# nvpro-samples/vk_gltf_renderer

Measured on AMD Instinct MI355X. Metric: Msamples/s (and ms/frame @ fixed spp) 1080p & 4K, 1/2/4/8 MI355X, higher is better.
Workload: dtype f32

## Files before the change

### include/mi_pt.h

```cpp
#ifndef MI_PT_H
#define MI_PT_H

#include "mi_pt_shaderio.h"

#ifdef __cplusplus
extern "C" {
#endif

#if defined(__GNUC__)
#define MI_PT_API __attribute__((visibility("default")))
#else
#define MI_PT_API
#endif

typedef enum MiPtStatus
{
  MI_PT_OK            = 0,
  MI_PT_ERR_ARGUMENT  = -1,
  MI_PT_ERR_NO_DEVICE = -2,
  MI_PT_ERR_HIP       = -3,
  MI_PT_ERR_STATE     = -4,
  MI_PT_ERR_IO        = -5
} MiPtStatus;

// ... 92 lines not shown
  int   bounceIterations;
  float tracePrimaryMs;
  float shadeFirstMs;
  int   tracePrimaryLaunches;
  int   shadeFirstLaunches;
} MiPtFrameTiming;

typedef struct MiPt MiPt;

MI_PT_API int mi_pt_create(const MiPtSceneDesc* scene, const MiPtCreateOptions* options, MiPt** out);

MI_PT_API int mi_pt_update_render_nodes(MiPt* pt, const MiGltfRenderNode* renderNodes, int numRenderNodes, const uint8_t* renderNodeVisible);

MI_PT_API int mi_pt_update_lights(MiPt* pt, const MiGltfLight* lights, int numLights);

MI_PT_API int mi_pt_update_materials(MiPt* pt, const MiGltfShadeMaterial* materials, int numMaterials, const MiGltfTextureInfo* textureInfos,
                                     int numTextureInfos);

typedef struct MiPtDeformPrimitive
{
  int32_t         renderPrimID;
  uint32_t        vertexCount;
  const float*    basePositions;
  const float*    baseNormals;
  const float*    baseTangents;
  const uint16_t* joints;
  const float*    weights;
  uint32_t        numJoints;
  uint32_t        jointMatrixOffset;
  uint32_t        numTargets;
  uint32_t        morphWeightOffset;
  const float*    positionDeltas;
  const float*    normalDeltas;
  const float*    tangentDeltas;
} MiPtDeformPrimitive;

typedef struct MiPtDeformDesc
{
  const MiPtDeformPrimitive* prims;
  int                        numPrims;
  int                        numJointMatrices;
  int                        numMorphWeights;
  const float*               jointMatrices;
  const float*               morphWeights;
} MiPtDeformDesc;

enum { MI_PT_DEFORM_DEFER_BUILD = 1 };

MI_PT_API int mi_pt_set_deformation(MiPt* pt, const MiPtDeformDesc* desc);
MI_PT_API int mi_pt_update_deformation(MiPt* pt, const float* jointMatrices, const float* morphWeights, int flags);
enum
{
  MI_PT_ACCEL_REBUILD = 0,
  MI_PT_ACCEL_REFIT   = 1,
  MI_PT_ACCEL_AUTO    = 2
};
enum { MI_PT_ACCEL_LAST_BUILD = 0, MI_PT_ACCEL_LAST_REFIT = 1 };
MI_PT_API int mi_pt_set_accel_update(MiPt* pt, int mode, float rebuildCostRatio);
typedef struct MiPtAccelInfo
{
  int32_t  mode;
  int32_t  lastUpdate;
  float    rebuildCostRatio;
  int32_t  reserved;
  uint64_t builds;
  uint64_t refits;
  double   sahCostAtBuild;
  double   sahCost;
  uint64_t trianglesMoved;
  uint64_t refitBytes;
} MiPtAccelInfo;
MI_PT_API int mi_pt_get_accel_info(MiPt* pt, MiPtAccelInfo* info);
MI_PT_API int mi_pt_set_accel_resident(MiPt* pt, int enable);
typedef struct MiPtAccelResidentInfo
{
  int32_t  enabled;
  int32_t  inForce;
  uint64_t residentTriangles;
  uint64_t hiddenTriangles;
  uint64_t visibilityRefits;
  uint64_t materialPatches;
} MiPtAccelResidentInfo;
MI_PT_API int mi_pt_get_accel_resident_info(MiPt* pt, MiPtAccelResidentInfo* info);
MI_PT_API int mi_pt_read_vertices(MiPt* pt, int renderPrimID, float* positions, float* normals, float* tangents);

MI_PT_API int mi_pt_destroy(MiPt* pt);

MI_PT_API int mi_pt_set_environment(MiPt* pt, const MiPtEnvironment* env);

MI_PT_API int mi_pt_resize(MiPt* pt, int width, int height);

MI_PT_API int mi_pt_set_frame_info(MiPt* pt, const MiSceneFrameInfo* info);
MI_PT_API int mi_pt_set_sky(MiPt* pt, const MiSkyPhysicalParameters* sky);

MI_PT_API int mi_pt_set_tile_partition(MiPt* pt, int rank, int world, int tileSize);

MI_PT_API int mi_pt_bind_accum(MiPt* pt, void* deviceRGBA32F);
MI_PT_API int mi_pt_bind_guides(MiPt* pt, void* deviceAlbedoRGBA32F, void* deviceNormalRGBA32F, void* deviceDepthR32F);

MI_PT_API int mi_pt_render_frame(MiPt* pt, const MiPathtraceParams* params, void* hipStream);

MI_PT_API int mi_pt_render_frames(MiPt* pt, const MiPathtraceParams* params, int numFrames, void* hipStream);

MI_PT_API int mi_pt_set_frame_queue(MiPt* pt, int depth);

MI_PT_API int mi_pt_synchronize(MiPt* pt);

MI_PT_API int mi_pt_read_accum(MiPt* pt, float* hostRGBA32F);
MI_PT_API int mi_pt_write_accum(MiPt* pt, const float* hostRGBA32F);
MI_PT_API int mi_pt_read_guides(MiPt* pt, float* hostAlbedoRGBA32F, float* hostNormalRGBA32F);
MI_PT_API int mi_pt_read_selection(MiPt* pt, uint32_t* hostObjectIds);
MI_PT_API int mi_pt_read_depth(MiPt* pt, float* hostDepth);
MI_PT_API void* mi_pt_accum_device_ptr(MiPt* pt);

MI_PT_API int mi_pt_denoise(MiPt* pt, int iterations, float sigmaColor, float sigmaNormal, float sigmaAlbedo,
                            float* hostRGBA32F, void* hipStream);

MI_PT_API int mi_pt_denoise_svgf(MiPt* pt, int iterations, float sigmaLuminance, float sigmaNormal, float sigmaDepth, float* hostRGBA32F, void* hipStream);


MI_PT_API int mi_pt_read_first_hit(MiPt* pt, float* hostXYZW);
MI_PT_API int mi_pt_set_temporal(MiPt* pt, int enable);
MI_PT_API int mi_pt_read_motion(MiPt* pt, float* hostRGBA32F);
typedef struct MiPtTemporalParams
{
  int   iterations;
  float sigmaLuminance;
  float sigmaNormal;
  float sigmaDepth;
  float alpha;
  float momentsAlpha;
  float maxHistory;
  float normalCos;
  float depthTolerance;
} MiPtTemporalParams;
MI_PT_API void mi_pt_default_temporal(MiPtTemporalParams* params);
MI_PT_API int mi_pt_denoise_temporal(MiPt* pt, const MiPtTemporalParams* params, float* hostRGBA32F, void* hipStream);
MI_PT_API int mi_pt_reset_history(MiPt* pt);

MI_PT_API int mi_pt_set_vertex_motion(MiPt* pt, int enable);
MI_PT_API int mi_pt_read_first_hit_triangle(MiPt* pt, uint32_t* hostPrimTriB1B2);
MI_PT_API int mi_pt_read_previous_positions(MiPt* pt, int renderPrimID, float* positions);

enum { MI_PT_VERTICES_RECOMPUTE_NORMALS = 1 };
typedef struct MiPtVertexUpdate
{
  int32_t      renderPrimID;
  uint32_t     vertexCount;
  const float* positions;
  const float* normals;
  const float* tangents;
  uint32_t     reserved[2];
} MiPtVertexUpdate;
MI_PT_API int mi_pt_set_vertex_updates(MiPt* pt, const int32_t* renderPrimIDs, int count, int flags);
MI_PT_API int mi_pt_update_vertices(MiPt* pt, const MiPtVertexUpdate* updates, int numUpdates, int flags);
MI_PT_API int mi_pt_update_vertices_device(MiPt* pt, const MiPtVertexUpdate* updates, int numUpdates, int flags);
typedef struct MiPtVertexUpdateInfo
{
  uint64_t calls;
  uint64_t verticesWritten;
  uint64_t verticesRejected;
  uint64_t tableBytes;
} MiPtVertexUpdateInfo;
MI_PT_API int mi_pt_get_vertex_update_info(MiPt* pt, MiPtVertexUpdateInfo* info);

typedef struct MiPtRay
// ... 83 lines not shown
```

### vk_gltf_renderer_amd/_capi.py

```python
import ctypes as C
import os
from enum import IntEnum

_HERE = os.path.dirname(os.path.abspath(__file__))
LIB_DIR = os.path.join(_HERE, "lib")

f32 = C.c_float
i32 = C.c_int
u32 = C.c_uint32


class MiGltfRenderNode(C.Structure):
    _fields_ = [("objectToWorld", f32 * 16), ("worldToObject", f32 * 16), ("materialID", i32), ("renderPrimID", i32)]


class MiGltfLight(C.Structure):
    _fields_ = [("direction", f32 * 3), ("type", i32), ("position", f32 * 3), ("radius", f32), ("color", f32 * 3),
                ("intensity", f32), ("angularSizeOrInvRange", f32), ("innerAngle", f32), ("outerAngle", f32), ("_pad", i32)]


class MiGltfTextureInfo(C.Structure):
    _fields_ = [("uvTransform", f32 * 6), ("index", i32), ("texCoord", i32)]


# ... 43 lines not shown
                ("sunGlowIntensity", f32), ("yIsUp", i32)]


class MiEnvAccel(C.Structure):
    _fields_ = [("alias", u32), ("q", f32)]


class MiTonemapperData(C.Structure):
    _fields_ = [("method", i32), ("isActive", i32), ("exposure", f32), ("brightness", f32), ("contrast", f32), ("saturation", f32), ("vignette", f32),
                ("autoExposure", i32), ("autoExposureSpeed", f32), ("evMinValue", f32), ("evMaxValue", f32), ("enableCenterMetering", i32)]


TONEMAP_METHODS = ("filmic", "uncharted", "clip", "aces", "agx", "khronos_pbr")


class MiPtRenderPrimitive(C.Structure):
    _fields_ = [("indices", C.POINTER(u32)), ("triangleCount", u32), ("vertexCount", u32), ("positions", C.POINTER(f32)),
                ("normals", C.POINTER(f32)), ("colors", C.POINTER(u32)), ("tangents", C.POINTER(f32)),
                ("texCoords0", C.POINTER(f32)), ("texCoords1", C.POINTER(f32)), ("opaqueTriangleCount", u32), ("reserved", u32)]


class MiPtTexture(C.Structure):
    _fields_ = [("levels", C.POINTER(C.POINTER(C.c_uint8))), ("width", i32), ("height", i32), ("numLevels", i32),
                ("srgb", i32), ("magFilter", i32), ("minFilter", i32), ("mipmapMode", i32), ("wrapS", i32), ("wrapT", i32)]


class MiPtSceneDesc(C.Structure):
    _fields_ = [("materials", C.POINTER(MiGltfShadeMaterial)), ("numMaterials", i32),
                ("textureInfos", C.POINTER(MiGltfTextureInfo)), ("numTextureInfos", i32),
                ("renderNodes", C.POINTER(MiGltfRenderNode)), ("numRenderNodes", i32),
                ("renderNodeVisible", C.POINTER(C.c_uint8)),
                ("renderPrimitives", C.POINTER(MiPtRenderPrimitive)), ("numRenderPrimitives", i32),
                ("lights", C.POINTER(MiGltfLight)), ("numLights", i32),
                ("textures", C.POINTER(MiPtTexture)), ("numTextures", i32)]


class MiPtEnvironment(C.Structure):
    _fields_ = [("rgba", C.POINTER(f32)), ("accel", C.POINTER(MiEnvAccel)), ("width", i32), ("height", i32), ("integral", f32)]


class MiPtCreateOptions(C.Structure):
    _fields_ = [("device", i32), ("collectCounters", i32), ("bvhBuilder", i32), ("reserved", i32 * 5)]


class MiPtStats(C.Structure):
    _fields_ = [(n, C.c_uint64) for n in (
        "cameraPaths", "segments", "shadowRays", "nodesClosest", "trisClosest", "nodesShadow", "trisShadow",
        "textureTaps", "bvhNodeCount", "bvhTriangleCount", "bvhNodeBytes", "bvhTriangleBytes", "surfaceHits", "nodesPrimary", "trisPrimary")]


class MiPtMemory(C.Structure):
    _fields_ = [(n, C.c_uint64) for n in ("sceneBytes", "rendererBytes", "deviceUsedBytes", "deviceTotalBytes", "pathStateBytes", "pathSlots")]


class MiPtFrameTiming(C.Structure):
    _fields_ = [("totalMs", f32), ("generateMs", f32), ("traceClosestMs", f32), ("sortMs", f32), ("shadeMs", f32),
                ("traceShadowMs", f32), ("accumulateMs", f32), ("traceClosestLaunches", i32), ("shadeLaunches", i32),
                ("traceShadowLaunches", i32), ("bounceIterations", i32), ("tracePrimaryMs", f32), ("shadeFirstMs", f32),
                ("tracePrimaryLaunches", i32), ("shadeFirstLaunches", i32)]


class MiPtDeformPrimitive(C.Structure):
    _fields_ = [("renderPrimID", i32), ("vertexCount", u32), ("basePositions", C.POINTER(f32)), ("baseNormals", C.POINTER(f32)),
                ("baseTangents", C.POINTER(f32)), ("joints", C.POINTER(C.c_uint16)), ("weights", C.POINTER(f32)), ("numJoints", u32),
                ("jointMatrixOffset", u32), ("numTargets", u32), ("morphWeightOffset", u32), ("positionDeltas", C.POINTER(f32)),
                ("normalDeltas", C.POINTER(f32)), ("tangentDeltas", C.POINTER(f32))]


class MiPtDeformDesc(C.Structure):
    _fields_ = [("prims", C.POINTER(MiPtDeformPrimitive)), ("numPrims", i32), ("numJointMatrices", i32), ("numMorphWeights", i32),
                ("jointMatrices", C.POINTER(f32)), ("morphWeights", C.POINTER(f32))]


class MiPtAccelInfo(C.Structure):
    _fields_ = [("mode", i32), ("lastUpdate", i32), ("rebuildCostRatio", f32), ("reserved", i32), ("builds", C.c_uint64), ("refits", C.c_uint64),
                ("sahCostAtBuild", C.c_double), ("sahCost", C.c_double), ("trianglesMoved", C.c_uint64), ("refitBytes", C.c_uint64)]


class MiPtAccelResidentInfo(C.Structure):
    _fields_ = [("enabled", i32), ("inForce", i32), ("residentTriangles", C.c_uint64), ("hiddenTriangles", C.c_uint64),
                ("visibilityRefits", C.c_uint64), ("materialPatches", C.c_uint64)]


class MiPtTemporalParams(C.Structure):
    _fields_ = [("iterations", i32), ("sigmaLuminance", f32), ("sigmaNormal", f32), ("sigmaDepth", f32), ("alpha", f32), ("momentsAlpha", f32),
                ("maxHistory", f32), ("normalCos", f32), ("depthTolerance", f32)]


class MiPtRay(C.Structure):
    _fields_ = [("origin", f32 * 3), ("tMin", f32), ("direction", f32 * 3), ("tMax", f32)]


class MiPtRayHit(C.Structure):
    _fields_ = [("t", f32), ("b1", f32), ("b2", f32), ("flags", u32), ("renderNode", i32), ("renderPrimID", i32), ("triangle", u32),
                ("materialID", i32), ("position", f32 * 3), ("reserved0", f32), ("normal", f32 * 3), ("reserved1", f32)]


class MiPtQueryOptions(C.Structure):
    _fields_ = [("mode", i32), ("alpha", i32), ("cull", i32), ("maxHits", i32), ("blendThreshold", f32), ("seed", u32), ("reserved", i32 * 2)]


class MiPtVertexUpdate(C.Structure):
    _fields_ = [("renderPrimID", i32), ("vertexCount", u32), ("positions", C.c_void_p), ("normals", C.c_void_p), ("tangents", C.c_void_p),
                ("reserved", u32 * 2)]


class MiPtVertexUpdateInfo(C.Structure):
    _fields_ = [(n, C.c_uint64) for n in ("calls", "verticesWritten", "verticesRejected", "tableBytes")]


class MiCamera(C.Structure):
    _fields_ = [("eye", f32 * 3), ("center", f32 * 3), ("up", f32 * 3), ("fovDegrees", f32), ("znear", f32),
                ("zfar", f32), ("orthographic", i32), ("xmag", f32), ("ymag", f32)]


assert C.sizeof(MiGltfRenderNode) == 136
assert C.sizeof(MiGltfLight) == 64
assert C.sizeof(MiGltfTextureInfo) == 32
assert C.sizeof(MiGltfShadeMaterial) == 288
assert C.sizeof(MiSceneFrameInfo) == 396
assert C.sizeof(MiPtAccelInfo) == 64
assert C.sizeof(MiPtAccelResidentInfo) == 40
assert C.sizeof(MiPtRay) == 32
assert C.sizeof(MiPtRayHit) == 64
assert C.sizeof(MiPtQueryOptions) == 32
assert C.sizeof(MiPtVertexUpdate) == 40
assert C.sizeof(MiPtVertexUpdateInfo) == 32

MI_PT_ABI_VERSION = 9
MI_PT_DEFORM_DEFER_BUILD = 1
MI_PT_VERTICES_RECOMPUTE_NORMALS = 1
(MI_SCENE_CHANGED_NODES, MI_SCENE_CHANGED_LIGHTS, MI_SCENE_CHANGED_DEFORMATION, MI_SCENE_CHANGED_MATERIALS, MI_SCENE_CHANGED_CAMERAS,
 MI_SCENE_CHANGED_VISIBILITY) = 1, 2, 4, 8, 16, 32
MI_PT_ACCEL_REBUILD, MI_PT_ACCEL_REFIT, MI_PT_ACCEL_AUTO = 0, 1, 2
MI_PT_ACCEL_LAST_BUILD, MI_PT_ACCEL_LAST_REFIT = 0, 1
MI_PT_HIT, MI_PT_HIT_FRONT_FACE, MI_PT_HIT_INVALID_RAY = 1, 2, 4
MI_PT_QUERY_CLOSEST, MI_PT_QUERY_ANY, MI_PT_QUERY_NEAREST_K = 0, 1, 2
MI_PT_QUERY_ALPHA_OPAQUE, MI_PT_QUERY_ALPHA_CUTOFF, MI_PT_QUERY_ALPHA_STOCHASTIC = 0, 1, 2
MI_PT_QUERY_CULL_NONE, MI_PT_QUERY_CULL_MATERIAL = 0, 1
MI_PT_QUERY_MAX_HITS = 8
MI_PT_CAMERA_RAYS_UNIT = 1
MI_PROJECTION_PERSPECTIVE, MI_PROJECTION_EQUIRECT, MI_PROJECTION_FISHEYE = 0, 1, 2
MI_PT_USE_DLSS, MI_PT_USE_OPTIX_DENOISER, MI_PT_FIRST_FRAME = 1, 2, 4
MI_SCENE_IS_ORTHOGRAPHIC, MI_SCENE_USE_SOLID_BACKGROUND, MI_SCENE_USE_HDR_ENVIRONMENT = 1, 2, 4
MI_SCENE_USE_INFINITE_PLANE, MI_SCENE_INFINITE_PLANE_SHADOW_CATCHER = 8, 16
MI_LIGHT_NONE, MI_LIGHT_DIRECTIONAL, MI_LIGHT_SPOT, MI_LIGHT_POINT = 0, 1, 2, 3


class Visualization(IntEnum):
    RENDERED = 0
    BASE_COLOR = 1
    METALLIC = 2
    ROUGHNESS = 3
    NORMAL_SHADING = 4
    NORMAL_GEOMETRIC = 5
    TANGENT = 6
    BITANGENT = 7
    EMISSIVE = 8
    OPACITY = 9
    TEXCOORD0 = 10
    TEXCOORD1 = 11
    CLAY = 12
    TRIANGLE_ID = 13
    FACE_ORIENTATION = 14
    OCCLUSION = 15
    CLEARCOAT_FACTOR = 16
    CLEARCOAT_ROUGHNESS = 17
    CLEARCOAT_NORMAL = 18
    SHEEN_COLOR = 19
    SHEEN_ROUGHNESS = 20
    SPECULAR_FACTOR = 21
    SPECULAR_COLOR = 22
    TRANSMISSION_FACTOR = 23
    IRIDESCENCE_FACTOR = 24
    IRIDESCENCE_THICKNESS = 25
    ANISOTROPY_STRENGTH = 26
    DIFFUSE_TRANSMISSION_FACTOR = 27
    DIFFUSE_TRANSMISSION_COLOR = 28
    OPACITY_MICROMAP = 29


MI_VIZ_COUNT = 30

P = C.POINTER
VP = C.c_void_p

HOST_SYMBOLS = {
    "mi_scene_load": (i32, [C.c_char_p, P(VP)]),
    "mi_scene_destroy": (None, [VP]),
    "mi_scene_desc": (P(MiPtSceneDesc), [VP]),
    "mi_scene_num_cameras": (i32, [VP]),
    "mi_scene_camera": (i32, [VP, i32, P(MiCamera)]),
    "mi_scene_bounds": (None, [VP, P(f32), P(f32)]),
    "mi_scene_num_triangles": (C.c_uint64, [VP]),
    "mi_hdr_load": (i32, [C.c_char_p, P(VP)]),
    "mi_scene_recompute_tangents": (i32, [VP, i32, i32]),
    "mi_mikktspace": (i32, [P(f32), P(f32), P(f32), u32, P(u32), u32, P(f32)]),
    "mi_scene_cut_alpha": (C.c_int64, [VP, i32]),
    "mi_scene_num_variants": (i32, [VP]),
    "mi_scene_variant_name": (i32, [VP, i32, C.c_char_p, i32]),
    "mi_scene_current_variant": (i32, [VP]),
    "mi_scene_set_variant": (i32, [VP, i32]),
    "mi_scene_num_animations": (i32, [VP]),
    "mi_scene_animation_info": (i32, [VP, i32, P(f32), P(f32), C.c_char_p, i32]),
    "mi_scene_update_animation": (i32, [VP, i32, f32]),
    "mi_scene_animation_changes": (i32, [VP]),
    "mi_scene_deformation": (P(MiPtDeformDesc), [VP]),
    "mi_scene_deform_on_host": (i32, [VP]),
    "mi_hdr_from_pixels": (i32, [i32, i32, P(f32), P(VP)]),
    "mi_hdr_destroy": (None, [VP]),
    "mi_hdr_env": (P(MiPtEnvironment), [VP]),
    "mi_default_sky": (None, [P(MiSkyPhysicalParameters)]),
    "mi_default_params": (None, [P(MiPathtraceParams)]),
    "mi_camera_frame_info": (None, [P(MiCamera), i32, i32, P(MiSceneFrameInfo), P(f32), P(f32)]),
    "mi_camera_rays": (i32, [P(MiCamera), i32, f32, i32, i32, P(f32), i32, P(MiPtRay), P(f32)]),
    "mi_host_last_error": (C.c_char_p, []),
}

PT_SYMBOLS = {
    "mi_pt_create": (i32, [P(MiPtSceneDesc), P(MiPtCreateOptions), P(VP)]),
    "mi_pt_destroy": (i32, [VP]),
    "mi_pt_set_environment": (i32, [VP, P(MiPtEnvironment)]),
    "mi_pt_resize": (i32, [VP, i32, i32]),
    "mi_pt_set_frame_info": (i32, [VP, P(MiSceneFrameInfo)]),
    "mi_pt_set_sky": (i32, [VP, P(MiSkyPhysicalParameters)]),
    "mi_pt_set_tile_partition": (i32, [VP, i32, i32, i32]),
    "mi_pt_bind_accum": (i32, [VP, VP]),
    "mi_pt_bind_guides": (i32, [VP, VP, VP, VP]),
    "mi_pt_render_frame": (i32, [VP, P(MiPathtraceParams), VP]),
    "mi_pt_render_frames": (i32, [VP, P(MiPathtraceParams), i32, VP]),
    "mi_pt_synchronize": (i32, [VP]),
    "mi_pt_read_accum": (i32, [VP, P(f32)]),
    "mi_pt_write_accum": (i32, [VP, P(f32)]),
    "mi_pt_read_guides": (i32, [VP, P(f32), P(f32)]),
    "mi_pt_read_selection": (i32, [VP, P(u32)]),
    "mi_pt_read_depth": (i32, [VP, P(f32)]),
    "mi_pt_set_frame_queue": (i32, [VP, i32]),
    "mi_pt_accum_device_ptr": (VP, [VP]),
    "mi_pt_denoise": (i32, [VP, i32, f32, f32, f32, P(f32), VP]),
    "mi_pt_denoise_svgf": (i32, [VP, i32, f32, f32, f32, P(f32), VP]),
    "mi_pt_denoised_device_ptr": (VP, [VP]),
    "mi_pt_tonemap": (i32, [VP, P(MiTonemapperData), i32, f32, P(C.c_uint8), VP]),
    "mi_pt_tonemapped_device_ptr": (VP, [VP]),
    "mi_pt_default_tonemapper": (None, [P(MiTonemapperData), i32]),
    "mi_pt_get_memory": (i32, [VP, P(MiPtMemory)]),
    "mi_pt_get_stats": (i32, [VP, P(MiPtStats)]),
    "mi_pt_reset_stats": (i32, [VP]),
    "mi_pt_enable_timing": (i32, [VP, i32]),
    "mi_pt_get_frame_timing": (i32, [VP, P(MiPtFrameTiming)]),
    "mi_pt_last_error": (C.c_char_p, []),
    "mi_pt_version": (C.c_char_p, []),
    "mi_pt_abi_version": (i32, []),
    "mi_pt_update_render_nodes": (i32, [VP, P(MiGltfRenderNode), i32, P(C.c_uint8)]),
    "mi_pt_update_lights": (i32, [VP, P(MiGltfLight), i32]),
    "mi_pt_update_materials": (i32, [VP, P(MiGltfShadeMaterial), i32, P(MiGltfTextureInfo), i32]),
    "mi_pt_set_deformation": (i32, [VP, P(MiPtDeformDesc)]),
    "mi_pt_update_deformation": (i32, [VP, P(f32), P(f32), i32]),
    "mi_pt_read_vertices": (i32, [VP, i32, P(f32), P(f32), P(f32)]),
    "mi_pt_set_accel_update": (i32, [VP, i32, f32]),
    "mi_pt_get_accel_info": (i32, [VP, P(MiPtAccelInfo)]),
    "mi_pt_set_accel_resident": (i32, [VP, i32]),
    "mi_pt_get_accel_resident_info": (i32, [VP, P(MiPtAccelResidentInfo)]),
    "mi_pt_read_first_hit": (i32, [VP, P(f32)]),
    "mi_pt_set_temporal": (i32, [VP, i32]),
    "mi_pt_read_motion": (i32, [VP, P(f32)]),
    "mi_pt_default_temporal": (None, [P(MiPtTemporalParams)]),
    "mi_pt_denoise_temporal": (i32, [VP, P(MiPtTemporalParams), P(f32), VP]),
    "mi_pt_reset_history": (i32, [VP]),
    "mi_pt_set_vertex_motion": (i32, [VP, i32]),
    "mi_pt_read_first_hit_triangle": (i32, [VP, P(u32)]),
    "mi_pt_read_previous_positions": (i32, [VP, i32, P(f32)]),
    "mi_pt_query_rays": (i32, [VP, P(MiPtRay), i32, i32, P(MiPtRayHit)]),
    "mi_pt_query_rays_device": (i32, [VP, VP, i32, i32, VP, VP]),
    "mi_pt_pick": (i32, [VP, P(f32), i32, P(MiPtRayHit)]),
    "mi_pt_default_query_options": (None, [P(MiPtQueryOptions)]),
    "mi_pt_query_rays_ex": (i32, [VP, P(MiPtRay), i32, P(MiPtQueryOptions), P(MiPtRayHit)]),
    "mi_pt_query_rays_device_ex": (i32, [VP, VP, i32, P(MiPtQueryOptions), VP, VP]),
    "mi_pt_pick_ex": (i32, [VP, P(f32), i32, P(MiPtQueryOptions), P(MiPtRayHit)]),
    "mi_pt_set_vertex_updates": (i32, [VP, P(i32), i32, i32]),
    "mi_pt_update_vertices": (i32, [VP, P(MiPtVertexUpdate), i32, i32]),
    "mi_pt_update_vertices_device": (i32, [VP, P(MiPtVertexUpdate), i32, i32]),
    "mi_pt_get_vertex_update_info": (i32, [VP, P(MiPtVertexUpdateInfo)]),
    "mi_pt_set_camera_rays": (i32, [VP, P(MiPtRay), i32, u32]),
    "mi_pt_set_camera_rays_device": (i32, [VP, VP, i32, u32]),
    "mi_pt_make_camera_rays": (i32, [VP, P(MiPathtraceParams), i32, P(MiPtRay)]),
    "mi_pt_make_camera_rays_device": (i32, [VP, P(MiPathtraceParams), i32, VP, VP]),
}


def _bind(lib, table):
    for name, (res, args) in table.items():
        fn = getattr(lib, name)
        fn.restype = res
        fn.argtypes = args
    return lib


_host = None
_pt = None


def host_lib():
    global _host
    if _host is None:
        path = os.path.join(LIB_DIR, "libmi_host.so")
        if not os.path.exists(path):
            raise RuntimeError(f"{path} is missing: run __graft_entry__.build() (make -C vk_gltf_renderer_amd/csrc)")
        _host = _bind(C.CDLL(path), HOST_SYMBOLS)
    return _host


def pt_lib():
    global _pt
    if _pt is None:
        path = os.environ.get("MI_PT_LIB") or os.path.join(LIB_DIR, "libmi_pt.so")
        if not os.path.exists(path):
            raise RuntimeError(f"{path} is missing: the HIP extension was not built; the product path has no fallback")
        _pt = _bind(C.CDLL(path), PT_SYMBOLS)
        if _pt.mi_pt_abi_version() != MI_PT_ABI_VERSION:
            raise RuntimeError(f"{path}: ABI version {_pt.mi_pt_abi_version()}, this binding was written for {MI_PT_ABI_VERSION}")
    return _pt


def device_source_id():
    import glob
    import hashlib
    root = os.path.dirname(_HERE)
    dev = os.path.join(_HERE, "csrc", "device")
    files = sorted(glob.glob(os.path.join(dev, "*.hip")) + glob.glob(os.path.join(dev, "*.h")), key=os.path.basename)
    files += [os.path.join(root, "include", "mi_pt.h"), os.path.join(root, "include", "mi_pt_shaderio.h")]
    h = hashlib.sha1()
    for f in files:
        h.update(open(f, "rb").read())
    return h.hexdigest()[:16]
```

### vk_gltf_renderer_amd/csrc/device/mi_pt_api.hip

```cpp
#include <hip/hip_runtime.h>

#include <algorithm>
#include <chrono>
#include <cstdlib>
#include <cmath>
#include <cstdio>
#include <cstring>
#include <memory>
#include <string>
#include <vector>

#include "mi_pt.h"
#include "bvh_refit.h"
#include "dev_buf.h"
#include "material_patch.h"
#include "pt_build.h"
#include "pt_bvh.h"
#include "pt_deform.h"
#include "pt_vertex_update.h"
#include "pt_kernels.h"
#include "pt_query.h"

namespace {

thread_local std::string g_lastError;

int fail(int code, const std::string& msg)
{
  g_lastError = msg;
  return code;
}

#define HIP_TRY(x)                                                                                                       \
  do                                                                                                                    \
  {                                                                                                                     \
    hipError_t e_ = (x);                                                                                                \
    if(e_ != hipSuccess)                                                                                                \
      return fail(MI_PT_ERR_HIP, std::string(#x) + ": " + hipGetErrorString(e_));                                       \
  } while(0)

using pt::DevBuf;

enum TimedKernel { TK_GENERATE, TK_TRACE, TK_SORT, TK_SHADE, TK_SHADOW, TK_ACCUM, TK_PRIMARY, TK_SHADE_FIRST, TK_COUNT };

}

struct RunSwitches
{
  int    packetInterval = 1;
  int    sortMode       = 2;
  bool   noPacket       = false;
  bool   stateBySlot    = false;
  bool   traceSpans     = false;
  int    overlapUpTo    = 32;
  int    overlapMinTris = 200000;
  bool   noPlanes       = false;
  bool   noOpaqueTris   = false;
  bool   noQuads        = false;
  bool   shadowFarFirst = true;
  int    reinsert       = 16;
  int    reinsertUpdate = 0;
  int    reinsertRounds = 4;
  float  splitFactor    = 4.0f;
  int    splitMaxDepth  = 8;
  float  splitMinShare  = 0.1f;
  bool   collapseGreedy = false;
  bool   collapseBad    = false;
  bool   hostCollapse   = false;
  bool   coreTex        = true;
  bool   shadowDeposit  = true;
  int    maxItersDiag   = 0;
  int    failBuildAt    = 0;
  bool   candPoolSet    = false;
  size_t candPool       = 0;
  void   read()
  {
    auto flag = [](const char* n) { const char* e = getenv(n); return e != nullptr; };
    auto num  = [](const char* n, int d) { const char* e = getenv(n); return e ? atoi(e) : d; };
    packetInterval = num("MI_PT_PACKET_INTERVAL", 1);
    sortMode       = num("MI_PT_SORT", 2);
    noPacket       = flag("MI_PT_NO_PACKET");
    stateBySlot    = flag("MI_PT_STATE_BY_SLOT");
    traceSpans     = flag("MI_PT_TRACE_SPANS");
    overlapUpTo    = num("MI_PT_OVERLAP", 32);
    overlapMinTris = num("MI_PT_OVERLAP_MIN_TRIS", 200000);
    noPlanes       = flag("MI_PT_DIAG_NO_PLANES");
    noOpaqueTris   = flag("MI_PT_DIAG_NO_OPAQUE_TRIS");
    noQuads        = flag("MI_PT_DIAG_NO_QUADS");
    shadowFarFirst = num("MI_PT_SHADOW_FAR_FIRST", 1) != 0;
    reinsert       = std::max(0, num("MI_PT_REINSERT", 16));
    reinsertUpdate = std::max(0, num("MI_PT_REINSERT_UPDATE", 0));
    reinsertRounds = std::max(1, num("MI_PT_REINSERT_ROUNDS", 4));
    if(const char* e = getenv("MI_PT_SPLIT"))
      splitFactor = std::max(0.0f, float(atof(e)));
    if(const char* e = getenv("MI_PT_SPLIT_MIN_SHARE"))
      splitMinShare = std::max(0.0f, float(atof(e)));
    splitMaxDepth  = std::min(std::max(0, num("MI_PT_SPLIT_DEPTH", 8)), 10);
    if(const char* e = getenv("MI_PT_COLLAPSE"))
    {
      collapseGreedy = strcmp(e, "greedy") == 0;
      collapseBad    = !collapseGreedy && strcmp(e, "sah") != 0;
    }
    hostCollapse   = flag("MI_PT_HOST_COLLAPSE");
    maxItersDiag   = num("MI_PT_DIAG_MAX_ITERS", 0);
    coreTex        = num("MI_PT_CORE_TEX", 1) != 0;
    shadowDeposit  = num("MI_PT_SHADOW_DEPOSIT", 1) != 0;
    failBuildAt    = num("MI_PT_DIAG_FAIL_BUILD", 0);
    if(const char* e = getenv("MI_PT_DIAG_CAND_POOL"))
    {
      candPoolSet = true;
      candPool    = size_t(strtoull(e, nullptr, 10));
    }
  }
};

struct MiPt
{
  int device = 0;
  int numCUs = 256;
  RunSwitches sw;
  int accelBuilds = 0;
  int               frameQueueDepth = 1;
  int               pendingFrames   = 0;
  MiPathtraceParams pendingFirst{};
  void*             pendingStream   = nullptr;
  DevBuf<MiGltfShadeMaterial> materials;
  DevBuf<MiGltfTextureInfo>   texInfos;
  DevBuf<pt::DevTexRef>       texRefs;
  DevBuf<pt::DevCoreTex>      coreTex;
  DevBuf<MiGltfRenderNode>    nodes;
  DevBuf<pt::DevPrim>         prims;
  DevBuf<MiGltfLight>         lights;
  DevBuf<pt::DevTexture>      textures;
  DevBuf<uchar4>              texels;
  DevBuf<uint4>               texQuads;
  DevBuf<uint8_t>             geometry;
  DevBuf<uint8_t>             instFlags;
  DevBuf<float>               srgbLut;
  DevBuf<float4>              envPixels;
  DevBuf<MiEnvAccel>          envAccel;
  DevBuf<pt::DevAlphaTri>     alphaTris;
  DevBuf<pt::DevShadeTri>     shadeTris;
  DevBuf<float4>              bvhNodes;
  DevBuf<uint4>               bvh8Nodes;
  DevBuf<float>               bvh8Planes;
  DevBuf<pt::DevTri>          bvhTris;
  bool                        wide      = true;
  pt::DevScene                scene{};
  bool                        hasAlpha = false, hasAlphaTest = false, hasVolumeScatter = false, simpleMaterials = true, hasTransmissive = false;
  static constexpr int        FC_RING = 32;
  DevBuf<pt::DevScene>        sceneDev;
  bool                        sceneDevDirty = true;
  DevBuf<pt::FrameConsts>     fcRing;
  DevBuf<pt::SkyPrecomp>      skyPre;
  MiSkyPhysicalParameters     skyPreFor{};
  bool                        skyPreValid = false;
  pt::FrameConsts*            fcHost = nullptr;
  hipEvent_t                  fcDone[FC_RING] = {};
  unsigned                    fcCursor = 0;
  MiPtStats                   staticStats{};
  std::vector<MiGltfRenderNode> hostNodes;
  std::vector<uint8_t>          hostVisible;
  std::vector<uint8_t>          matInstFlags;
  std::vector<uint8_t>          matFeatures;
  std::vector<MiGltfShadeMaterial> hostMaterials;
  std::vector<MiGltfTextureInfo>   hostTexInfos;
  std::vector<pt::DevTexture>      hostTextures;
  DevBuf<uint8_t>               matDirty;
  bool                          splitRefs = false;
  std::vector<uint32_t>         primTriangles;
  std::vector<pt::DevPrim>      hostPrims;
  std::vector<uint32_t>         primVertices;
  DevBuf<uint8_t>               deformPool;
  DevBuf<pt::DeformTask>        deformTasks;
  DevBuf<uint32_t>              deformBlockTask;
  DevBuf<float4>                deformJoints;
  DevBuf<float>                 deformWeights;
  int                           deformJointCount = 0, deformWeightCount = 0;
  uint32_t                      deformBlocks = 0;
  bool                          deformSet = false;
  std::vector<int>              deformPrimIDs;
  bool                          vuSet = false;
  std::vector<int>              vuPrimIDs;
  std::vector<uint8_t>          vuDeclared;
  std::vector<size_t>           vuCornerEnd, vuCorners;
  DevBuf<uint32_t>              vuTable;
  DevBuf<pt::VertexUpdateTask>  vuTasks;
  DevBuf<pt::NormalRebuildTask> vuNormalTasks;
  DevBuf<uint32_t>              vuBlockTask;
  size_t                        vuBlockCap = 0;
  DevBuf<uint8_t>               vuStaging;
  uint64_t                      vuCalls = 0, vuWritten = 0, vuRejected = 0;
  int                           bvhBuilder = 0;
  int                           accelMode = MI_PT_ACCEL_REBUILD;
  float                         accelRatio = 1.5f;
  int                           lastUpdate = MI_PT_ACCEL_LAST_BUILD;
  bool                          switchBuild = false;
  bool                          refitCapable = false;
  uint64_t                      accelRefits = 0, trianglesMoved = 0;
  double                        sahAtBuild = 0.0, sahNow = 0.0;
  DevBuf<pt::RefitBox>          refitSlotBox, refitBuiltBox, refitNodeBox;
  DevBuf<float>                 refitSah;
  DevBuf<double>                refitSahPartial;
  DevBuf<uint8_t>               refitDirty;
  std::vector<uint32_t>         refitLevels;
  std::vector<MiGltfRenderNode> builtNodes;
  std::vector<uint8_t>          primDirty;
  std::vector<uint8_t>          primDeformed;
  bool                          accelResident = false;
  bool                          residentTree  = false;
  uint64_t                      hiddenTris = 0;
  uint64_t                      visibilityRefits = 0, materialPatches = 0;
  int                     width = 0, height = 0;
  int                     tileRank = 0, tileWorld = 1, tileSize = 64;
  MiSceneFrameInfo        frameInfo{};
  MiSkyPhysicalParameters sky{};
  bool                    haveFrameInfo = false;
  DevBuf<uint32_t>        ownedTiles;
  int                     numSlots = 0, tilesX = 0, tilesY = 0;
  int                     framesCap = 1;
  size_t                  queueCap  = 0;
  DevBuf<float4>          pathArrays;
  DevBuf<float4>          optThroughput, optMisc, optMedium, optPixelSum, optGuides, optShadowAux2;
  DevBuf<float4>          firstHit;
  pt::PathSoA             paths{};
  DevBuf<uint32_t>        queueMem;
  DevBuf<float4>          queuePayload;
  DevBuf<float4>          candPool;
  DevBuf<uint32_t>        candLists;
  pt::Queues              queues{};
  DevBuf<float4>          accumOwn, albedo, normal, denoiseA, denoiseB;
  float4*                 albedoBound = nullptr;
// ... 1049 lines not shown
          if(p.normals) { o[3] = p.normals[3 * size_t(v)]; o[4] = p.normals[3 * size_t(v) + 1]; o[5] = p.normals[3 * size_t(v) + 2]; }
          if(p.texCoords0) { o[6] = p.texCoords0[2 * size_t(v)]; o[7] = p.texCoords0[2 * size_t(v) + 1]; }
          if(p.tangents) memcpy(o + 8, p.tangents + 4 * size_t(v), 16);
        }
        d.verts = reinterpret_cast<const float4*>(put(iv.data(), iv.size() * sizeof(float)));
      }
    }
    HIP_TRY(hipMemcpy(pt->geometry.ptr, staging.data(), staging.size(), hipMemcpyHostToDevice));
  }
  HIP_TRY(pt->prims.upload(devPrims.data(), devPrims.size()));
  pt->hostPrims = devPrims;
  for(int i = 0; i < sd->numRenderPrimitives; ++i)
    pt->primVertices.push_back(sd->renderPrimitives[i].vertexCount);
  phase("tables + geometry upload");

  pt->hostNodes.assign(sd->renderNodes, sd->renderNodes + sd->numRenderNodes);
  if(sd->renderNodeVisible)
    pt->hostVisible.assign(sd->renderNodeVisible, sd->renderNodeVisible + sd->numRenderNodes);
  pt->matInstFlags.resize(size_t(sd->numMaterials));
  pt->matFeatures.resize(size_t(sd->numMaterials));
  pt->hostMaterials.assign(sd->materials, sd->materials + sd->numMaterials);
  pt->hostTexInfos.assign(sd->textureInfos, sd->textureInfos + sd->numTextureInfos);
  for(int m = 0; m < sd->numMaterials; ++m)
  {
    pt->matInstFlags[size_t(m)] = materialInstFlags(sd->materials[m]);
    pt->matFeatures[size_t(m)]  = materialFeatures(sd->materials[m]);
  }
  pt->primTriangles.resize(size_t(sd->numRenderPrimitives));
  for(int i = 0; i < sd->numRenderPrimitives; ++i)
  {
    const MiPtRenderPrimitive& rp = sd->renderPrimitives[i];
    pt->primTriangles[size_t(i)]  = (rp.positions && rp.indices) ? rp.triangleCount : 0u;
  }
  pt->bvhBuilder = options ? options->bvhBuilder : 0;

  {
    std::vector<pt::DevTexture> dt(size_t(sd->numTextures));
    size_t                      totalTexels = 0;
    for(int i = 0; i < sd->numTextures; ++i)
    {
      const MiPtTexture& t = sd->textures[i];
      if(t.numLevels < 1 || t.numLevels > 16 || t.width < 1 || t.height < 1 || t.width > 65535 || t.height > 65535)
        return fail(MI_PT_ERR_ARGUMENT, "mi_pt_create: texture dimensions / level count out of range");
      for(int l = 0; l < t.numLevels; ++l)
        totalTexels += size_t(std::max(1, t.width >> l)) * size_t(std::max(1, t.height >> l));
    }
    if(totalTexels > 0xffffffffull)
      return fail(MI_PT_ERR_ARGUMENT, "mi_pt_create: texture pool exceeds 2^32 texels");
    std::vector<uchar4> pool(std::max<size_t>(totalTexels, 1));
    size_t              off = 0;
    for(int i = 0; i < sd->numTextures; ++i)
    {
      const MiPtTexture& t = sd->textures[i];
      pt::DevTexture&    d = dt[size_t(i)];
      memset(&d, 0, sizeof(d));
      d.width = uint16_t(t.width); d.height = uint16_t(t.height); d.numLevels = uint8_t(t.numLevels); d.srgb = uint8_t(t.srgb ? 1 : 0);
      d.magFilter = uint8_t(t.magFilter); d.minFilter = uint8_t(t.minFilter); d.mipmapMode = uint8_t(t.mipmapMode);
      d.wrapS = uint8_t(t.wrapS); d.wrapT = uint8_t(t.wrapT);
      for(int l = 0; l < t.numLevels; ++l)
      {
        size_t n         = size_t(std::max(1, t.width >> l)) * size_t(std::max(1, t.height >> l));
        d.levelOffset[l] = uint32_t(off);
        memcpy(&pool[off], t.levels[l], n * 4);
        off += n;
      }
    }
    HIP_TRY(pt->textures.upload(dt.data(), dt.size()));
    HIP_TRY(pt->texels.upload(pool.data(), pool.size()));
    if(totalTexels > 0 && !pt->sw.noQuads)
    {
      HIP_TRY(pt->texQuads.alloc(pool.size()));
      for(const pt::DevTexture& d : dt)
        for(int l = 0; l < d.numLevels; ++l)
          pt::launchTextureQuads(pt->texels.ptr, pt->texQuads.ptr, d.levelOffset[l], std::max(1, int(d.width) >> l), std::max(1, int(d.height) >> l), d.wrapS,
                                 d.wrapT, nullptr);
      HIP_TRY(hipGetLastError());
    }
    pt->hostTextures = dt;
    std::vector<pt::DevTexRef>  refs;
    std::vector<pt::DevCoreTex> core;
    deriveTextureRecords(pt.get(), sd->materials, sd->numMaterials, sd->textureInfos, sd->numTextureInfos, refs, core);
    HIP_TRY(pt->texRefs.upload(refs.data(), refs.size()));
    HIP_TRY(pt->coreTex.upload(core.data(), core.size()));
  }
  {
    float lut[256];
    for(int i = 0; i < 256; ++i)
    {
      float c = float(i) / 255.0f;
      lut[i]  = c <= 0.04045f ? c / 12.92f : std::pow((c + 0.055f) / 1.055f, 2.4f);
    }
    HIP_TRY(pt->srgbLut.upload(lut, 256));
  }
  phase("textures upload");

  pt::DevScene& S = pt->scene;
  S.materials = pt->materials.ptr; S.texInfos = pt->texInfos.ptr; S.nodes = pt->nodes.ptr; S.prims = pt->prims.ptr; S.lights = pt->lights.ptr;
  S.textures = pt->textures.ptr; S.texels = pt->texels.ptr; S.texQuads = pt->texQuads.ptr; S.envPixels = nullptr; S.envAccel = nullptr; S.bvhNodes = nullptr; S.bvh8Nodes = nullptr; S.bvh8Planes = nullptr; S.tris = nullptr;
  S.geomPool = reinterpret_cast<const float4*>(pt->geometry.ptr);
  S.texRefs = pt->texRefs.ptr; S.coreTex = reinterpret_cast<const uint4*>(pt->coreTex.ptr); S.alphaTris = nullptr; S.shadeTris = nullptr; S.srgbLut = pt->srgbLut.ptr; S.numMaterials = sd->numMaterials; S.numTextures = sd->numTextures;
  S.numLights = sd->numLights; S.numNodes = sd->numRenderNodes;
  S.envWidth = 0; S.envHeight = 0;
  S.packetInterval = pt->sw.packetInterval;
  S.shadowOctFlip  = pt->sw.shadowFarFirst ? 7u : 0u;
  if(int rc = buildAcceleration(pt.get()))
    return rc;
  phase("shade / alpha records");
  HIP_TRY(pt->stats.alloc(1));
  HIP_TRY(hipMemset(pt->stats.ptr, 0, sizeof(pt::StatCounters)));
  MiSkyPhysicalParameters s{};
  s.rgbUnitConversion[0] = s.rgbUnitConversion[1] = s.rgbUnitConversion[2] = 1.0f / 80000.0f;
  s.multiplier = 0.1f; s.haze = 0.1f; s.redblueshift = 0.1f; s.saturation = 1.0f; s.groundColor[0] = s.groundColor[1] = s.groundColor[2] = 0.4f;
  s.horizonBlur = 0.3f; s.sunDiskIntensity = 1.0f; s.sunDirection[0] = s.sunDirection[1] = s.sunDirection[2] = 0.5773502691896258f;
  s.sunDiskScale = 1.0f; s.sunGlowIntensity = 1.0f; s.yIsUp = 1;
  pt->sky = s;
  *out    = pt.release();
  return MI_PT_OK;
}

int mi_pt_update_render_nodes(MiPt* pt, const MiGltfRenderNode* renderNodes, int numRenderNodes, const uint8_t* renderNodeVisible)
{
  FLUSH_PENDING(pt);
  if(!pt || !renderNodes || numRenderNodes != int(pt->hostNodes.size()))
    return fail(MI_PT_ERR_ARGUMENT, "mi_pt_update_render_nodes: the render-node count must be the one the instance was created with");
  for(int n = 0; n < numRenderNodes; ++n)
    if(renderNodes[n].materialID >= int(pt->matInstFlags.size()))
      return fail(MI_PT_ERR_ARGUMENT, "mi_pt_update_render_nodes: render node references a material beyond the table");
  if(residentInForce(pt))
    return updateRenderNodesResident(pt, renderNodes, numRenderNodes, renderNodeVisible);
  HIP_TRY(hipSetDevice(pt->device));
  HIP_TRY(hipDeviceSynchronize());
  bool                 sameTopology = true;
  std::vector<uint8_t> moved(size_t(numRenderNodes), 0);
  for(int n = 0; n < numRenderNodes; ++n)
  {
    const MiGltfRenderNode &was = pt->hostNodes[size_t(n)], &now = renderNodes[n];
    const bool              visWas = pt->hostVisible.empty() || pt->hostVisible[size_t(n)], visNow = !renderNodeVisible || renderNodeVisible[n];
    if(was.materialID != now.materialID || was.renderPrimID != now.renderPrimID || visWas != visNow)
      sameTopology = false;
    moved[size_t(n)] = memcmp(was.objectToWorld, now.objectToWorld, sizeof(float) * 32) != 0;
  }
  pt->hostNodes.assign(renderNodes, renderNodes + numRenderNodes);
  if(renderNodeVisible)
    pt->hostVisible.assign(renderNodeVisible, renderNodeVisible + numRenderNodes);
  else
    pt->hostVisible.clear();
  return updateAcceleration(pt, sameTopology, moved);
}

int mi_pt_update_lights(MiPt* pt, const MiGltfLight* lights, int numLights)
{
  FLUSH_PENDING(pt);
  if(!pt || numLights != pt->scene.numLights || (numLights > 0 && !lights))
    return fail(MI_PT_ERR_ARGUMENT, "mi_pt_update_lights: the light count must be the one the instance was created with");
  if(numLights == 0)
    return MI_PT_OK;
  HIP_TRY(hipSetDevice(pt->device));
  HIP_TRY(hipDeviceSynchronize());
  HIP_TRY(hipMemcpy(pt->lights.ptr, lights, sizeof(MiGltfLight) * size_t(numLights), hipMemcpyHostToDevice));
  return MI_PT_OK;
}

int mi_pt_update_materials(MiPt* pt, const MiGltfShadeMaterial* materials, int numMaterials, const MiGltfTextureInfo* textureInfos, int numTextureInfos)
{
  FLUSH_PENDING(pt);
  if(!pt || !materials || !textureInfos || numMaterials != int(pt->hostMaterials.size()))
    return fail(MI_PT_ERR_ARGUMENT, "mi_pt_update_materials: the material count must be the one the instance was created with");
  if(numTextureInfos <= 0)
    return fail(MI_PT_ERR_ARGUMENT, "mi_pt_update_materials: the texture-info table needs the reserved slot 0");
  {
    std::string why;
    if(!materialSlotsInRange(materials, numMaterials, numTextureInfos, why))
      return fail(MI_PT_ERR_ARGUMENT, "mi_pt_update_materials: " + why);
  }
  const size_t         nm = size_t(numMaterials);
  std::vector<uint8_t> newFlags(nm), newFeatures(nm), alphaChanged(nm, 0), flagsChanged(nm, 0);
  bool                 anyAlpha = false, anyFlags = false, transmissiveChanged = false;
  for(size_t m = 0; m < nm; ++m)
  {
    newFlags[m]    = materialInstFlags(materials[m]);
    newFeatures[m] = materialFeatures(materials[m]);
    const AlphaKey was = alphaKey(pt->hostMaterials[m], pt->hostTexInfos.data()), now = alphaKey(materials[m], textureInfos);
    alphaChanged[m] = memcmp(&was, &now, sizeof(AlphaKey)) != 0;
    flagsChanged[m] = newFlags[m] != pt->matInstFlags[m];
    anyAlpha |= alphaChanged[m] != 0;
    anyFlags |= flagsChanged[m] != 0;
  }
  const int numNodes = int(pt->hostNodes.size()), numPrims = int(pt->hostPrims.size());
  auto      materialOf = [&](int n) { return size_t(std::max(0, std::min(pt->hostNodes[size_t(n)].materialID, numMaterials - 1))); };
  for(int n = 0; n < numNodes; ++n)
  {
    const size_t m    = materialOf(n);
    const int    prim = pt->hostNodes[size_t(n)].renderPrimID;
    if(alphaChanged[m] && prim >= 0 && prim < numPrims && pt->hostPrims[size_t(prim)].opaqueTriangles > 0)
      return fail(MI_PT_ERR_ARGUMENT, "mi_pt_update_materials: alpha state of a material whose geometry was cut at load: re-cut and re-create (material "
                                          + std::to_string(m) + ", render node " + std::to_string(n) + ")");
    if(((newFlags[m] ^ pt->matInstFlags[m]) & pt::INST_TRANSMISSIVE) != 0)
      transmissiveChanged = true;
  }
  HIP_TRY(hipSetDevice(pt->device));
  HIP_TRY(hipDeviceSynchronize());
  {
    std::vector<pt::DevTexRef>  refs;
    std::vector<pt::DevCoreTex> core;
    deriveTextureRecords(pt, materials, numMaterials, textureInfos, numTextureInfos, refs, core);
    if(size_t(numTextureInfos) != pt->texInfos.count)
    {
      DevBuf<MiGltfTextureInfo> infos;
      DevBuf<pt::DevTexRef>     drefs;
      HIP_TRY(infos.upload(textureInfos, size_t(numTextureInfos)));
      HIP_TRY(drefs.upload(refs.data(), refs.size()));
      std::swap(pt->texInfos.ptr, infos.ptr); std::swap(pt->texInfos.count, infos.count);
      std::swap(pt->texRefs.ptr, drefs.ptr); std::swap(pt->texRefs.count, drefs.count);
      pt->scene.texInfos = pt->texInfos.ptr;
      pt->scene.texRefs  = pt->texRefs.ptr;
    }
    else
    {
      HIP_TRY(hipMemcpy(pt->texInfos.ptr, textureInfos, sizeof(MiGltfTextureInfo) * size_t(numTextureInfos), hipMemcpyHostToDevice));
      HIP_TRY(hipMemcpy(pt->texRefs.ptr, refs.data(), sizeof(pt::DevTexRef) * refs.size(), hipMemcpyHostToDevice));
    }
    HIP_TRY(hipMemcpy(pt->materials.ptr, materials, sizeof(MiGltfShadeMaterial) * nm, hipMemcpyHostToDevice));
    HIP_TRY(hipMemcpy(pt->coreTex.ptr, core.data(), sizeof(pt::DevCoreTex) * core.size(), hipMemcpyHostToDevice));
  }
  pt->hostMaterials.assign(materials, materials + numMaterials);
  pt->hostTexInfos.assign(textureInfos, textureInfos + numTextureInfos);
  pt->matInstFlags = newFlags;
  pt->matFeatures  = newFeatures;
  pt->sceneDevDirty = true;
  const bool hadTransmissive = pt->hasTransmissive, wasSimple = pt->simpleMaterials;
  const std::vector<uint8_t> flags = instanceFlags(pt);
  if((anyAlpha || anyFlags) && pt->scene.numTris > 0 && (!pt->wide || (transmissiveChanged && pt->splitRefs)))
  {
    if(int rc = buildAcceleration(pt))
      return rc;
    return followSummaries(pt, hadTransmissive, wasSimple);
  }
  if(pt->scene.numTris > 0)
  {
    std::vector<uint8_t> dirty(size_t(std::max(numNodes, 1)), 0);
    for(int n = 0; n < numNodes; ++n)
    {
      const size_t m = materialOf(n);
      dirty[size_t(n)] = uint8_t((flagsChanged[m] ? pt::MATERIAL_PATCH_FLAGS : 0) | (alphaChanged[m] ? pt::MATERIAL_PATCH_ALPHA : 0));
    }
    if(int rc = patchTriangleData(pt, flags, dirty))
      return rc;
  }
  return followSummaries(pt, hadTransmissive, wasSimple);
}

static void releaseDeformation(MiPt* pt)
{
  pt->deformPool.release();
  pt->deformTasks.release();
  pt->deformBlockTask.release();
  pt->deformJoints.release();
  pt->deformWeights.release();
  pt->deformJointCount = pt->deformWeightCount = 0;
  pt->deformBlocks = 0;
  pt->deformSet    = false;
  pt->deformPrimIDs.clear();
}

int mi_pt_set_deformation(MiPt* pt, const MiPtDeformDesc* desc)
{
  FLUSH_PENDING(pt);
  if(!pt)
    return fail(MI_PT_ERR_ARGUMENT, "mi_pt_set_deformation: null instance");
  HIP_TRY(hipSetDevice(pt->device));
  HIP_TRY(hipDeviceSynchronize());
  if(!desc)
  {
    releaseDeformation(pt);
    return allocVertexMotion(pt);
  }
  const int numPrims = int(pt->primVertices.size());
  if(desc->numPrims < 0 || desc->numJointMatrices < 0 || desc->numMorphWeights < 0 || (desc->numPrims > 0 && !desc->prims))
    return fail(MI_PT_ERR_ARGUMENT, "mi_pt_set_deformation: negative count or null primitive table");
  std::vector<uint8_t> seen(size_t(numPrims), 0);
  size_t               poolBytes = 0;
  uint64_t             blocks    = 0;
  for(int k = 0; k < desc->numPrims; ++k)
  {
    const MiPtDeformPrimitive& d   = desc->prims[k];
    const std::string          who = "mi_pt_set_deformation: primitive " + std::to_string(k) + ": ";
    if(d.renderPrimID < 0 || d.renderPrimID >= numPrims)
      return fail(MI_PT_ERR_ARGUMENT, who + "render primitive " + std::to_string(d.renderPrimID) + " out of range");
    if(seen[size_t(d.renderPrimID)]++)
      return fail(MI_PT_ERR_ARGUMENT, who + "render primitive " + std::to_string(d.renderPrimID) + " listed twice");
    if(pt->vuSet && pt->vuDeclared[size_t(d.renderPrimID)])
      return fail(MI_PT_ERR_ARGUMENT, who + "render primitive " + std::to_string(d.renderPrimID) + " is driven by the caller (mi_pt_set_vertex_updates)");
    const pt::DevPrim& rp = pt->hostPrims[size_t(d.renderPrimID)];
    if(d.vertexCount != pt->primVertices[size_t(d.renderPrimID)])
      return fail(MI_PT_ERR_ARGUMENT, who + "vertexCount differs from the resident primitive's");
    if(!d.basePositions || !rp.positions)
      return fail(MI_PT_ERR_ARGUMENT, who + "no base positions");
    if((d.baseNormals && !rp.normals) || (d.baseTangents && !rp.tangents))
// ... 405 lines not shown
  if(!pt || !out)
    return fail(MI_PT_ERR_ARGUMENT, "mi_pt_get_vertex_update_info: null argument");
  out->calls            = pt->vuCalls;
  out->verticesWritten  = pt->vuWritten;
  out->verticesRejected = pt->vuRejected;
  out->tableBytes       = pt->vuTable.bytes();
  return MI_PT_OK;
}

int mi_pt_set_accel_update(MiPt* pt, int mode, float rebuildCostRatio)
{
  FLUSH_PENDING(pt);
  if(!pt)
    return fail(MI_PT_ERR_ARGUMENT, "mi_pt_set_accel_update: null instance");
  if(mode != MI_PT_ACCEL_REBUILD && mode != MI_PT_ACCEL_REFIT && mode != MI_PT_ACCEL_AUTO)
    return fail(MI_PT_ERR_ARGUMENT, "mi_pt_set_accel_update: unknown mode " + std::to_string(mode));
  if(!std::isfinite(rebuildCostRatio) || rebuildCostRatio < 1.0f)
    return fail(MI_PT_ERR_ARGUMENT, "mi_pt_set_accel_update: the rebuild cost ratio must be finite and at least 1");
  HIP_TRY(hipSetDevice(pt->device));
  HIP_TRY(hipDeviceSynchronize());
  pt->accelMode  = mode;
  pt->accelRatio = rebuildCostRatio;
  if(mode == MI_PT_ACCEL_REBUILD)
  {
    releaseRefitData(pt);
    return MI_PT_OK;
  }
  if(!pt->refitLevels.empty() || !pt->refitCapable)
    return MI_PT_OK;
  pt->switchBuild = true;
  const int rc    = buildAcceleration(pt);
  pt->switchBuild = false;
  return rc;
}

int mi_pt_get_accel_info(MiPt* pt, MiPtAccelInfo* out)
{
  if(!pt || !out)
    return fail(MI_PT_ERR_ARGUMENT, "mi_pt_get_accel_info: null argument");
  memset(out, 0, sizeof(*out));
  out->mode             = pt->accelMode;
  out->lastUpdate       = pt->lastUpdate;
  out->rebuildCostRatio = pt->accelRatio;
  out->builds           = uint64_t(std::max(pt->accelBuilds, 0));
  out->refits           = pt->accelRefits;
  out->sahCostAtBuild   = pt->sahAtBuild;
  out->sahCost          = pt->sahNow;
  out->trianglesMoved   = pt->trianglesMoved;
  out->refitBytes       = refitBytes(pt);
  return MI_PT_OK;
}

int mi_pt_set_accel_resident(MiPt* pt, int enable)
{
  FLUSH_PENDING(pt);
  if(!pt)
    return fail(MI_PT_ERR_ARGUMENT, "mi_pt_set_accel_resident: null instance");
  HIP_TRY(hipSetDevice(pt->device));
  HIP_TRY(hipDeviceSynchronize());
  pt->accelResident = enable != 0;
  if(residentWanted(pt) == pt->residentTree || pt->accelMode == MI_PT_ACCEL_REBUILD || (pt->bvhBuilder & 1) != 0 || pt->sw.hostCollapse)
    return MI_PT_OK;
  pt->switchBuild = true;
  const int rc    = buildAcceleration(pt);
  pt->switchBuild = false;
  return rc;
}

int mi_pt_get_accel_resident_info(MiPt* pt, MiPtAccelResidentInfo* out)
{
  if(!pt || !out)
    return fail(MI_PT_ERR_ARGUMENT, "mi_pt_get_accel_resident_info: null argument");
  memset(out, 0, sizeof(*out));
  const bool inForce     = residentInForce(pt);
  out->enabled           = pt->accelResident ? 1 : 0;
  out->inForce           = inForce ? 1 : 0;
  out->residentTriangles = inForce ? uint64_t(std::max(pt->scene.numTris, 0)) : 0;
  out->hiddenTriangles   = inForce ? pt->hiddenTris : 0;
  out->visibilityRefits  = pt->visibilityRefits;
  out->materialPatches   = pt->materialPatches;
  return MI_PT_OK;
}

int mi_pt_read_vertices(MiPt* pt, int renderPrimID, float* positions, float* normals, float* tangents)
{
  FLUSH_PENDING(pt);
  if(!pt || renderPrimID < 0 || renderPrimID >= int(pt->hostPrims.size()))
    return fail(MI_PT_ERR_ARGUMENT, "mi_pt_read_vertices: no such render primitive");
  HIP_TRY(hipSetDevice(pt->device));
  HIP_TRY(hipDeviceSynchronize());
  const pt::DevPrim& p  = pt->hostPrims[size_t(renderPrimID)];
  const size_t       nv = pt->primVertices[size_t(renderPrimID)];
  if(positions && p.positions && nv)
    HIP_TRY(hipMemcpy(positions, p.positions, nv * 12, hipMemcpyDeviceToHost));
  if(normals && p.normals && nv)
    HIP_TRY(hipMemcpy(normals, p.normals, nv * 12, hipMemcpyDeviceToHost));
  if(tangents && p.tangents && nv)
    HIP_TRY(hipMemcpy(tangents, p.tangents, nv * 16, hipMemcpyDeviceToHost));
  return MI_PT_OK;
}

int mi_pt_destroy(MiPt* pt)
{
  if(pt)
    pt->pendingFrames = 0;
  if(!pt)
    return MI_PT_OK;
  (void)hipSetDevice(pt->device);
  (void)hipDeviceSynchronize();
  pt::dumpTraceProfile();
  delete pt;
  return MI_PT_OK;
}

int mi_pt_set_environment(MiPt* pt, const MiPtEnvironment* env)
{
  FLUSH_PENDING(pt);
  if(!pt)
    return fail(MI_PT_ERR_ARGUMENT, "mi_pt_set_environment: null instance");
  HIP_TRY(hipSetDevice(pt->device));
  HIP_TRY(hipDeviceSynchronize());
  if(!env || !env->rgba || !env->accel || env->width <= 0 || env->height <= 0)
  {
    pt->envPixels.release();
    pt->envAccel.release();
    pt->scene.envPixels = nullptr;
    pt->scene.envAccel  = nullptr;
    pt->scene.envWidth = pt->scene.envHeight = 0;
    pt->sceneDevDirty  = true;
    return MI_PT_OK;
  }
  const size_t n = size_t(env->width) * size_t(env->height);
  HIP_TRY(pt->envPixels.upload(reinterpret_cast<const float4*>(env->rgba), n));
  HIP_TRY(pt->envAccel.upload(env->accel, n));
  pt->scene.envPixels = pt->envPixels.ptr;
  pt->scene.envAccel  = pt->envAccel.ptr;
  pt->scene.envWidth  = env->width;
  pt->scene.envHeight = env->height;
  pt->sceneDevDirty   = true;
  return MI_PT_OK;
}

int mi_pt_resize(MiPt* pt, int width, int height)
{
  FLUSH_PENDING(pt);
  if(!pt || width <= 0 || height <= 0 || width > 32768 || height > 32768)
    return fail(MI_PT_ERR_ARGUMENT, "mi_pt_resize: need 0 < width, height <= 32768");
  HIP_TRY(hipSetDevice(pt->device));
  HIP_TRY(hipDeviceSynchronize());
  pt->width       = width;
  pt->height      = height;
  pt->denoised    = nullptr;
  pt->accumFrames = 0.0f;
  pt->momentFrames = 0.0f;
  return allocFrameResources(pt);
}

int mi_pt_set_frame_info(MiPt* pt, const MiSceneFrameInfo* info)
{
  if(!pt || !info)
    return fail(MI_PT_ERR_ARGUMENT, "mi_pt_set_frame_info: null argument");
  if(pt->haveFrameInfo && memcmp(&pt->frameInfo, info, sizeof(*info)) == 0)
    return MI_PT_OK;
  FLUSH_PENDING(pt);
  pt->frameInfo     = *info;
  pt->haveFrameInfo = true;
// ... 108 lines not shown
    return fail(MI_PT_ERR_ARGUMENT, "mi_pt_render_frame: numSamples >= 1 and 1 <= maxDepth <= 255 required");
  if((pt->frameInfo.flags & MI_SCENE_USE_HDR_ENVIRONMENT) && !pt->scene.envPixels)
    return fail(MI_PT_ERR_STATE, "mi_pt_render_frame: HDR environment requested but none was set");
  if(cameraRaysStale(pt))
    return fail(MI_PT_ERR_STATE, CAMERA_RAYS_STALE);
  HIP_TRY(hipSetDevice(pt->device));
  hipStream_t stream = reinterpret_cast<hipStream_t>(hipStream);
  pt->lastStream     = stream;
  if(pt->numSlots == 0)
    return MI_PT_OK;
  if(numFrames > pt->framesCap)
  {
    HIP_TRY(hipDeviceSynchronize());
    if(int rc = allocPathResources(pt, numFrames))
      return rc;
  }

  pt::LaunchCtx c;
  c.scene = pt->scene;
  memset(&c.fc, 0, sizeof(c.fc));
  c.fc.frameInfo = pt->frameInfo;
  c.fc.sky       = pt->sky;
  if(!pt->skyPreValid || memcmp(&pt->skyPreFor, &pt->sky, sizeof(pt->sky)) != 0)
  {
    if(!pt->skyPre.ptr)
      HIP_TRY(pt->skyPre.alloc(1));
    pt::launchSkyPrecomp(pt->sky, pt->skyPre.ptr, stream);
    pt->skyPreFor   = pt->sky;
    pt->skyPreValid = true;
  }
  c.fc.skyPre    = pt->skyPre.ptr;
  c.fc.pc        = *params;
  c.fc.width     = pt->width;
  c.fc.height    = pt->height;
  c.fc.tileSize  = pt->tileSize;
  c.fc.tileShift = 0;
  while((1 << c.fc.tileShift) < pt->tileSize)
    ++c.fc.tileShift;
  c.fc.numSlots  = pt->numSlots;
  c.fc.numFrames = numFrames;
  pt::divideMagic(uint32_t(std::max(numFrames, 2)), c.fc.framesMagic, c.fc.framesShift);
  c.fc.slotLayout = numFrames % 64 == 0 ? 1 : 0;
  c.fc.stateInQueue = (!pt->sw.stateBySlot && !(pt->frameInfo.flags & MI_SCENE_INFINITE_PLANE_SHADOW_CATCHER)) ? 1 : 0;
  const bool guides = (params->flags & MI_PT_USE_OPTIX_DENOISER) != 0;
  if(int rc = ensureOptionalPathArrays(pt, c.fc.stateInQueue == 0, params->numSamples > 1, guides, (pt->frameInfo.flags & MI_SCENE_INFINITE_PLANE_SHADOW_CATCHER) != 0))
    return rc;
  c.paths        = pt->paths;
  {
    const bool stateBySlot = c.fc.stateInQueue == 0, multiSample = params->numSamples > 1;
    if(!(stateBySlot || multiSample))
      c.paths.misc = nullptr;
    if(!stateBySlot)
      c.paths.throughput = nullptr;
    if(!multiSample)
      c.paths.pixelSum = nullptr;
  }
  pt->accumFrames   = float(params->totalSamples) / float(params->numSamples) + float(numFrames);
  if(guides && (params->totalSamples == 0 || pt->momentFrames == pt->accumFrames - float(numFrames)))
    pt->momentFrames = pt->accumFrames;
  else if(!guides || params->totalSamples == 0)
    pt->momentFrames = 0.0f;
  if(!guides)
  {
    c.paths.guideAlbedo = nullptr;
    c.paths.guideNormal = nullptr;
  }
  c.queues           = pt->queues;
  if(!(pt->frameInfo.flags & MI_SCENE_INFINITE_PLANE_SHADOW_CATCHER))
    c.queues.shadow.aux2 = nullptr;
  c.ownedTiles       = pt->ownedTiles.ptr;
  c.stats            = pt->stats.ptr;
  c.stream           = stream;
  c.persistentBlocks = unsigned(pt->numCUs) * 8u;
  c.hasAlpha         = pt->hasAlpha;
  c.hasAlphaClosest  = c.hasAlpha && pt->hasAlphaTest;
  c.visualization    = pt->frameInfo.visualization > MI_VIZ_RENDERED && pt->frameInfo.visualization < MI_VIZ_COUNT;
  if(pt->frameInfo.visualization == MI_VIZ_OPACITY_MICROMAP)
    c.hasAlphaClosest = false;
  c.hasTransmissive  = pt->hasTransmissive;
  c.simpleMaterials  = pt->simpleMaterials;
  c.wide             = pt->wide;
  c.collectCounters  = pt->collectCounters;
  c.shadowDeposit    = pt->sw.shadowDeposit;
  {
    c.sortMode = pt->sw.sortMode;
  }
  if(pt->sceneDevDirty)
  {
    HIP_TRY(hipDeviceSynchronize());
    HIP_TRY(pt->sceneDev.upload(&pt->scene, 1));
    pt->sceneDevDirty = false;
  }
  if(!pt->fcHost)
  {
    HIP_TRY(hipHostMalloc(reinterpret_cast<void**>(&pt->fcHost), sizeof(pt::FrameConsts) * MiPt::FC_RING, hipHostMallocDefault));
    HIP_TRY(pt->fcRing.alloc(MiPt::FC_RING));
    for(hipEvent_t& e : pt->fcDone)
      HIP_TRY(hipEventCreateWithFlags(&e, hipEventDisableTiming));
  }
  const unsigned fcSlot = pt->fcCursor++ % unsigned(MiPt::FC_RING);
  if(pt->fcCursor > unsigned(MiPt::FC_RING))
    HIP_TRY(hipEventSynchronize(pt->fcDone[fcSlot]));
  pt->fcHost[fcSlot] = c.fc;
  HIP_TRY(hipMemcpyAsync(pt->fcRing.ptr + fcSlot, pt->fcHost + fcSlot, sizeof(pt::FrameConsts), hipMemcpyHostToDevice, stream));
  c.sceneDev = pt->sceneDev.ptr;
  c.fcDev    = pt->fcRing.ptr + fcSlot;

  auto timedOn = [&](hipStream_t on, int kind, auto&& launch) {
    if(pt->timingEnabled)
    {
      hipEvent_t a = getEvent(pt, pt->evCursor), b = getEvent(pt, pt->evCursor);
      (void)hipEventRecord(a, on);
      launch();
      (void)hipEventRecord(b, on);
      pt->pendingSpans.push_back({kind, a, b});
    }
    else
      launch();
  };
  auto timed = [&](int kind, auto&& launch) { timedOn(stream, kind, launch); };
  hipEvent_t frameA = nullptr, frameB = nullptr;
  if(pt->timingEnabled)
  {
    frameA = getEvent(pt, pt->evCursor);
    frameB = getEvent(pt, pt->evCursor);
    (void)hipEventRecord(frameA, stream);
  }
  int iterations = 0, traceLaunches = 0, shadeLaunches = 0, shadowLaunches = 0;
  const bool usePacket = !pt->sw.noPacket;
  const bool debugSpans = pt->sw.traceSpans;
  bool overlap = pt->sw.overlapUpTo > 0 && ((numFrames <= pt->sw.overlapUpTo && pt->scene.numTris >= pt->sw.overlapMinTris) || pt->hasVolumeScatter)
                 && c.fc.stateInQueue != 0 && !debugSpans;
  if(overlap && !pt->sideStream)
    overlap = hipStreamCreateWithFlags(&pt->sideStream, hipStreamNonBlocking) == hipSuccess && hipEventCreateWithFlags(&pt->evShaded, hipEventDisableTiming) == hipSuccess
              && hipEventCreateWithFlags(&pt->evShadowed, hipEventDisableTiming) == hipSuccess;
  pt::LaunchCtx cSide = c;
  cSide.stream        = pt->sideStream;
  struct SideJoin
  {
    hipStream_t side        = nullptr;
    bool        outstanding = false;
    ~SideJoin()
    {
      if(outstanding && side)
        (void)hipStreamSynchronize(side);
    }
  } sideJoin;
  sideJoin.side = overlap ? pt->sideStream : nullptr;
  for(int s = 0; s < params->numSamples; ++s)
  {
    pt::launchResetCounters(c.queues, stream);
    const bool boundRays    = pt->cameraRays != nullptr;
    const bool fusedPrimary = c.wide && usePacket && !debugSpans && !boundRays;
    if(fusedPrimary)
    {
      timed(TK_PRIMARY, [&] { pt::launchTracePrimary(c, s); });
      if(pt->timingEnabled)
        ++pt->accTiming.tracePrimaryLaunches;
    }
    else if(boundRays)
      timed(TK_GENERATE, [&] { pt::launchGenerateRays(c, pt->cameraRays, uint32_t(pt->cameraRaySets), (pt->cameraRayFlags & MI_PT_CAMERA_RAYS_UNIT) != 0, s); });
    else
      timed(TK_GENERATE, [&] { pt::launchGenerate(c, s); });
    int cur = 0;
    int maxIters = params->maxDepth;
    if((pt->frameInfo.flags & MI_SCENE_USE_INFINITE_PLANE) && (pt->frameInfo.flags & MI_SCENE_INFINITE_PLANE_SHADOW_CATCHER))
// ... 874 lines not shown
```

### vk_gltf_renderer_amd/csrc/device/pt_kernels.h

```cpp
#pragma once
#include <hip/hip_runtime.h>

#include "pt_scene.h"
#include "pt_temporal.h"

namespace pt {

struct LaunchCtx
{
  DevScene        scene;
  FrameConsts     fc;
  const DevScene*    sceneDev;
  const FrameConsts* fcDev;
  PathSoA         paths;
  Queues          queues;
  const uint32_t* ownedTiles;
  StatCounters*   stats;
  hipStream_t     stream;
  unsigned        persistentBlocks;
  bool            hasAlpha;
  bool            hasAlphaClosest;
  bool            hasTransmissive;
  bool            simpleMaterials;
  bool            wide;
  bool            collectCounters;
  bool            shadowDeposit;
  int             sortMode;
  bool            visualization;
};

void launchBuildShadeRecords(const DevScene& scene, uint32_t numTris, DevShadeTri* out, hipStream_t s);
void launchBuildAlphaRecords(const DevScene& scene, uint32_t numTris, DevAlphaTri* out, hipStream_t s);
void launchPatchMaterials(const DevScene& scene, const uint8_t* instFlags, const uint8_t* dirty, DevTri* tris, DevAlphaTri* alphaTris, DevShadeTri* shadeTris,
                          uint32_t numTris, hipStream_t s);
void dumpTraceProfile();
void launchBvh8Planes(const uint4* nodes, uint32_t numNodes, float* planes, hipStream_t s);
void launchTextureQuads(const uchar4* texels, uint4* quads, uint32_t offset, int width, int height, int wrapS, int wrapT, hipStream_t s);
void launchResetCounters(const Queues& Q, hipStream_t s);
void launchSkyPrecomp(const MiSkyPhysicalParameters& sky, SkyPrecomp* out, hipStream_t stream);
void launchGenerate(const LaunchCtx& c, int sampleIndex);
void launchTraceClosest(const LaunchCtx& c, int cur);
void launchTracePrimary(const LaunchCtx& c, int sampleIndex);
void launchShade(const LaunchCtx& c, int cur, bool first);
void launchTraceShadow(const LaunchCtx& c, int nxt);
void launchFlushSurvivors(const LaunchCtx& c, int cur);
void launchFinishSample(const LaunchCtx& c, int sampleIndex, float4* accum, float* depth, float4* albedo, float4* normal);
void launchSelection(const LaunchCtx& c, uint32_t* selection);
void launchGenerateRays(const LaunchCtx& c, const MiPtRay* rays, uint32_t numSets, bool unit, int sampleIndex);
void launchSelectionRays(const LaunchCtx& c, const MiPtRay* rays, uint32_t set, uint32_t* selection);
void launchExportCameraRays(const LaunchCtx& c, MiPtRay* out, uint32_t setBase);
struct QueryRules;
void launchQueryRaysEx(const DevScene& scene, bool wide, bool any, const QueryRules& q, const MiPtRay* rays, uint32_t numRays, MiPtRayHit* hits, hipStream_t s);
void launchPickRaysEx(const DevScene& scene, const FrameConsts& fc, bool wide, const QueryRules& q, const float2* xy, MiPtRay* rayScratch, uint32_t numRays,
                      MiPtRayHit* hits, hipStream_t s);

void launchAtrous(const float4* in, float4* out, const float4* albedo, const float4* normal, int width, int height, int step, float sigmaColor,
                  float sigmaNormal, float sigmaAlbedo, hipStream_t s);

const float4* launchSvgf(const float4* color, const float4* albedo, const float4* normal, const float* depth, float4* bufA, float4* bufB, int width, int height,
                         int iterations, float frames, float sigmaLuminance, float sigmaNormal, float sigmaDepth, hipStream_t s);

const float4* launchSvgfFilter(float4* in, float4* other, const float4* color, const float4* albedo, const float4* normal, const float* depth, int width,
                               int height, int iterations, float sigmaLuminance, float sigmaNormal, float sigmaDepth, hipStream_t s);

void launchMotionVectors(const float4* firstHit, const uint4* firstHitTri, const VertexMotionPrim* vmPrims, int numPrims, const uint32_t* ownedTiles,
                         uint32_t numSlots, int tileShift, int width, int height, const MiGltfRenderNode* nodes, float* prevObjectToWorld, int numNodes,
                         const float* viewProj, const float* prevMVP, float4* motion, hipStream_t s);
void launchSnapshotTransforms(const MiGltfRenderNode* nodes, float* prevObjectToWorld, int numNodes, hipStream_t s);
void launchSnapshotPositions(const VertexMotionPrim* vmPrims, const uint32_t* ids, uint32_t numIds, uint32_t maxVertexCount, hipStream_t s);
void launchSvgfReproject(const float4* color, const float4* albedo, const float4* normal, const float* depth, const float4* motion, const TemporalHistory& in,
                         const TemporalHistory& out, float4* illum, int width, int height, const TemporalConsts& tc, bool haveHistory, hipStream_t s);

void launchTonemap(const float4* in, uint32_t* outRgba8, int width, int height, const MiTonemapperData& tm, uint32_t* histogram, float* autoState,
                   float dtSeconds, hipStream_t s);

}
```

### vk_gltf_renderer_amd/csrc/device/pt_kernels.hip

```cpp
#include <hip/hip_runtime.h>
#include <hip/hip_fp16.h>

#ifndef MI_PT_EXACT_FP
#define PT_FAST_SHADING_MATH 1
#endif
#include "pt_kernels.h"
#include "pt_shading.h"
#include "pt_bvh.h"
#include "pt_bvh8.h"
#include "pt_lane_walk.h"
#include "pt_camera.h"
#include "pt_packet.h"
#include "pt_feed.h"
#include "pt_visualize.h"

namespace pt {

namespace {

constexpr int TRACE_BLOCK = 1024;
#ifndef NODE_CACHE_EXTRA
#define NODE_CACHE_EXTRA 0
#endif
constexpr int NODE_CACHE  = 712 + NODE_CACHE_EXTRA;
// ... 1090 lines not shown
  }
  const uint32_t pos0 = (chunk % NSUB) * Q.subCap + (chunk / NSUB) * QCHUNK;
  if(toShade)
  {
    const uint32_t pos   = pos0 + before + laneCountBelow(shadeMask);
    Q.active[0].slot[pos] = slot;
    Q.active[0].org[pos]  = make_float4(cp.origin.x, cp.origin.y, cp.origin.z, 0.0f);
    Q.active[0].dir[pos]  = make_float4(cp.direction.x, cp.direction.y, cp.direction.z, __uint_as_float(cp.seed));
    Q.active[0].aux[pos]  = make_float4(best.t, __int_as_float(best.tri), best.u, best.v);
    const float4 misc0    = make_float4(0.0f, __uint_as_float(PF_ALIVE), __uint_as_float(cp.seed), 0.0f);
    if(fc.stateInQueue)
      Q.active[0].misc[pos] = misc0;
    else
      P.misc[slot] = misc0;
  }
  if(threadIdx.x >= total)
    Q.active[0].slot[pos0 + threadIdx.x] = QUEUE_DEAD;
  if(active && !toShade)
  {
    if(hasFlag(fc.pc.flags, MI_PT_FIRST_FRAME) && cp.frame == 0u)
      P.firstHit[pathSlotPixel(fc, slot)] = make_float4(cp.direction.x, cp.direction.y, cp.direction.z, 0.0f);
    P.radiance[slot] = make_float4(cp.direction.x, cp.direction.y, cp.direction.z, __uint_as_float(RADW_PRIMARY_MISS));
    if(P.guideAlbedo && fc.pc.numSamples == 1)
    {
      P.guideAlbedo[slot] = make_float4(0, 0, 0, 0);
      P.guideNormal[slot] = make_float4(0, 0, 0, 0);
    }
    if(P.misc)
      P.misc[slot] = make_float4(0.0f, __uint_as_float(PF_NOT_SOLID | PF_PRIMARY_MISS), __uint_as_float(cp.seed), 0.0f);
  }
  if(COUNT)
  {
    if(lane == 0)
    {
      atomicAdd(&stats->cameraPaths, (unsigned long long)__popcll(activeMask));
      atomicAdd(&stats->segments, (unsigned long long)__popcll(activeMask));
    }
    atomicAdd(&stats->nodesPrimary, (unsigned long long)nodes);
    atomicAdd(&stats->trisPrimary, (unsigned long long)tris);
  }
}

template <bool WIDE>
__global__ void __launch_bounds__(SEL_BLOCK) k_selection(DevScene sc, FrameConsts fc, const uint32_t* ownedTiles, uint32_t* selection)
{
  __shared__ int s_stack[BVH_STACK_LDS * SEL_BLOCK];
  uint32_t       slot = blockIdx.x * blockDim.x + threadIdx.x;
  int            px, py;
  if(slot >= uint32_t(fc.numSlots) || !slotToPixel(fc, ownedTiles, slot, px, py))
    return;
  f3 origin, direction;
  getRay(fc, mk2(float(px), float(py)), mk2(0.5f, 0.5f), origin, direction);
  const RaySetup r     = makeRaySetup(origin, direction);
  float          bestT = INFINITE_F;
  uint32_t       bestRnode = 0xffffffffu, bestPrim = 0xffffffffu;
  auto testTri = [&](int triIndex) {
    const DevTri T = sc.tris[triIndex];
    TriHit       h;
    if(!intersectTri(xyz(T.a), xyz(T.b), xyz(T.c), r.org, r.dir, h) || !(h.t > 0.0f))
      return false;
    const uint32_t rnode = __float_as_uint(T.a.w), prim = __float_as_uint(T.b.w);
    if(h.t < bestT || (h.t == bestT && (rnode < bestRnode || (rnode == bestRnode && prim < bestPrim))))
    {
      bestT = h.t; bestRnode = rnode; bestPrim = prim;
    }
    return true;
  };
  if(sc.bvhRoot != BVH_EMPTY)
    laneWalk<WIDE, false, SEL_BLOCK>(sc, r, bestT, s_stack, testTri, [&] { return bestT; });
  selection[size_t(py) * size_t(fc.width) + size_t(px)] = (bestRnode != 0xffffffffu) ? bestRnode + 1u : 0u;
}

template <bool COUNT, bool SIMPLE, bool FIRST>
__global__ void __launch_bounds__(SHADE_BLOCK, SIMPLE ? SHADE_SIMPLE_WAVES : 1) k_shade(const DevScene* __restrict__ scp, const FrameConsts* __restrict__ fcp, PathSoA P, Queues Q, int cur, int sortMode, StatCounters* stats)
{
  constexpr bool VIZ = false;
#include "pt_shade_body.h"
}
template <bool SIMPLE, bool FIRST>
__global__ void __launch_bounds__(SHADE_BLOCK, SIMPLE ? SHADE_SIMPLE_WAVES : 1) k_shade_viz(const DevScene* __restrict__ scp, const FrameConsts* __restrict__ fcp, PathSoA P, Queues Q, int cur, int sortMode, StatCounters* stats)
{
  constexpr bool COUNT = false, VIZ = true;
#include "pt_shade_body.h"
}

template <int MODE>
struct ShadowCfg
{
  static constexpr int BLOCK = MODE == 2 ? 256 : TRACE_BLOCK;
  static constexpr int CACHE = MODE == 2 ? 320 : (MODE == 1 ? NODE_CACHE_ALPHA : (MODE == 3 ? NODE_CACHE_ALPHA - 104 : NODE_CACHE));
};

PT_DEV void shadowDeposit(const PathSoA& P, const Queues& Q, int nxt, uint32_t slot, uint32_t qpos, bool catcherRay, f3 contrib, f3 total, bool occ,
                          float catcherDarken)
{
  if(!catcherRay)
  {
    if(!occ)
    {
      float4* const target = shadowTarget(P, Q, nxt, slot);
      float4        rad    = *target;
      rad.x += contrib.x * total.x;
      rad.y += contrib.y * total.y;
      rad.z += contrib.z * total.z;
      *target = rad;
    }
    return;
  }
  const float4 a2  = Q.shadow.aux2[qpos];
  const f3     sf  = occ ? mk3(0.0f) : total;
  float4       rad = P.radiance[slot];
  if(sf.x == 1.0f && sf.y == 1.0f && sf.z == 1.0f)
  {
    rad.x += a2.x; rad.y += a2.y; rad.z += a2.z;
    const uint32_t posNext = __float_as_uint(a2.w);
    if(posNext != 0xffffffffu)
      Q.active[nxt].slot[posNext] = QUEUE_DEAD;
  }
  else
  {
    f3 r3 = mk3(rad.x, rad.y, rad.z);
    r3 += contrib * sf;
    r3 -= contrib * (mk3(1.0f) - sf) * catcherDarken;
    rad.x = r3.x; rad.y = r3.y; rad.z = r3.z;
  }
  P.radiance[slot] = rad;
}

template <bool WIDE, int MODE, bool COUNT>
__global__ void __launch_bounds__(ShadowCfg<MODE>::BLOCK, TRACE_MIN_WAVES) k_trace_shadow(DevScene sc, const DevScene* __restrict__ scp, PathSoA P, Queues Q, int nxt, float catcherDarken, StatCounters* stats, int overflowOnly,
                                                                                          int walkDeposit)
{
  constexpr int  SBLOCK    = ShadowCfg<MODE>::BLOCK;
  constexpr bool HAS_ALPHA = MODE >= 1, HAS_TRANS = MODE == 2, REC = MODE == 3;
  constexpr bool DEFER = MODE == 1 || MODE == 3;
  const bool inWalk = !HAS_TRANS && !REC && walkDeposit != 0;
  constexpr bool LATE_CONTRIB = WIDE && MODE == 1;
  static_assert(!REC || WIDE, "the recording walk exists for the 8-wide BVH only");
  __shared__ int      s_stack[BVH_STACK_LDS * SBLOCK];
  __shared__ uint32_t s_prefix[NSUB + 1];
  __shared__ uint4    s_nodes[WIDE ? ShadowCfg<MODE>::CACHE * 5 : 1];
  __shared__ uint32_t s_items[(WIDE && !HAS_TRANS) ? SBLOCK : 1];
  __shared__ uint4    s_alpha[(WIDE && DEFER) ? SBLOCK : 1];
  __shared__ uint32_t s_head[REC ? SBLOCK : 1], s_ovf[REC ? SBLOCK : 1];
  __shared__ uint8_t  s_octLut[(WIDE && MI_PT_OCT_LUT) ? OCT_LUT_BYTES : 1];
  queuePrefix(&Q.counters[(nxt ? QC_PAIR1 : QC_PAIR0) + 1], s_prefix);
  const RayQueue in = Q.shadow;
  const bool     subset = MODE == 2 && overflowOnly != 0;
  uint32_t* const heads = &Q.counters[subset ? QC_HEADS_OVERFLOW : QC_HEADS_SHADOW];
  WaveFeed feed;
  feedInit(feed, subset ? Q.counters[QC_OVERFLOW] : s_prefix[NSUB]);
  if(!feedBlockHasWork(feed))
    return;
  if(WIDE && MI_PT_OCT_LUT)
    fillOctLut(s_octLut);
  const uint32_t cachedNodes = WIDE ? fillNodeCache(sc, s_nodes, uint32_t(ShadowCfg<MODE>::CACHE)) : 0u;
  LaneStack  st;
  LaneStack2 st2;
  int        stackOverflow[WIDE ? 2 * BVH8_STACK_PRIV : BVH_STACK_PRIV];
  st.lds = s_stack;  st.tid = int(threadIdx.x);  st.stride = SBLOCK;  st.sp = 0;  st.priv = stackOverflow;
  st2.lds = s_stack; st2.tid = int(threadIdx.x); st2.stride = SBLOCK; st2.sp = 0;
  st2.privBase = reinterpret_cast<uint32_t*>(stackOverflow); st2.privBits = reinterpret_cast<uint32_t*>(stackOverflow) + (WIDE ? BVH8_STACK_PRIV : 0);
  bool      active = false;
  uint32_t  slot   = 0;
  RaySetup  r{};
  int       node = BVH_EMPTY;
// ... 848 lines not shown
  const float darken = c.fc.frameInfo.shadowCatcherDarkenAmount;
  const bool  record = WIDE && c.hasAlpha && c.hasTransmissive && c.queues.candPool != nullptr;
  const int   mode   = !c.hasAlpha ? 0 : (c.hasTransmissive ? (record ? 3 : 2) : 1);
  const unsigned bs  = mode == 2 ? unsigned(ShadowCfg<2>::BLOCK) : unsigned(ShadowCfg<0>::BLOCK);
  dim3 grid(c.persistentBlocks * 256u / bs), block(bs);
#define MI_LAUNCH_SHADOW(M, C, OVF) \
  hipLaunchKernelGGL((k_trace_shadow<WIDE, M, C>), grid, block, 0, c.stream, c.scene, c.sceneDev, c.paths, c.queues, nxt, darken, c.stats, OVF, deposit)
  const int  deposit     = (c.shadowDeposit && (mode == 0 || mode == 1)) ? 1 : 0;
  const bool catcherRays = (c.fc.frameInfo.flags & MI_SCENE_USE_INFINITE_PLANE) && (c.fc.frameInfo.flags & MI_SCENE_INFINITE_PLANE_SHADOW_CATCHER);
  const dim3 rgrid(c.persistentBlocks), rblock(256);
  if(mode == 0)      { if(c.collectCounters) MI_LAUNCH_SHADOW(0, true, 0); else MI_LAUNCH_SHADOW(0, false, 0); }
  else if(mode == 1) { if(c.collectCounters) MI_LAUNCH_SHADOW(1, true, 0); else MI_LAUNCH_SHADOW(1, false, 0); }
  else if(mode == 2) { if(c.collectCounters) MI_LAUNCH_SHADOW(2, true, 0); else MI_LAUNCH_SHADOW(2, false, 0); }
  else
  {
    if constexpr(WIDE)
    {
      if(c.collectCounters) MI_LAUNCH_SHADOW(3, true, 0); else MI_LAUNCH_SHADOW(3, false, 0);
    }
  }
  if(mode == 3)
  {
    hipLaunchKernelGGL(k_shadow_resolve<true>, rgrid, rblock, 0, c.stream, c.sceneDev, c.paths, c.queues, nxt, darken, 0);
    if constexpr(WIDE)
    {
      grid  = dim3(c.persistentBlocks * 256u / unsigned(ShadowCfg<2>::BLOCK));
      block = dim3(unsigned(ShadowCfg<2>::BLOCK));
      if(c.collectCounters) MI_LAUNCH_SHADOW(2, true, 1); else MI_LAUNCH_SHADOW(2, false, 1);
    }
  }
  else if(mode != 2 && (!deposit || catcherRays))
    hipLaunchKernelGGL(k_shadow_resolve<false>, rgrid, rblock, 0, c.stream, c.sceneDev, c.paths, c.queues, nxt, darken, deposit);
#undef MI_LAUNCH_SHADOW
}
}
void launchTracePrimary(const LaunchCtx& c, int sampleIndex)
{
  const uint32_t batchSlots = uint32_t(c.fc.numSlots) * uint32_t(c.fc.numFrames);
  dim3           grid(batchSlots / 256u), block(256);
  const bool interval = c.fc.slotLayout == 1 && c.scene.packetInterval != 0 && c.scene.bvh8Planes != nullptr;
#define MI_LAUNCH_PRIMARY(A, C)                                                                                                                   \
  do                                                                                                                                              \
  {                                                                                                                                               \
    if(interval)                                                                                                                                  \
      hipLaunchKernelGGL((k_trace_primary<A, C, true>), grid, block, 0, c.stream, c.scene, c.fc, c.sceneDev, c.fcDev, c.paths, c.queues, c.ownedTiles, sampleIndex, batchSlots, c.stats);  \
    else                                                                                                                                          \
      hipLaunchKernelGGL((k_trace_primary<A, C, false>), grid, block, 0, c.stream, c.scene, c.fc, c.sceneDev, c.fcDev, c.paths, c.queues, c.ownedTiles, sampleIndex, batchSlots, c.stats); \
  } while(0)
  if(c.hasAlphaClosest)
  {
    if(c.collectCounters) MI_LAUNCH_PRIMARY(true, true); else MI_LAUNCH_PRIMARY(true, false);
  }
  else
  {
    if(c.collectCounters) MI_LAUNCH_PRIMARY(false, true); else MI_LAUNCH_PRIMARY(false, false);
  }
#undef MI_LAUNCH_PRIMARY
}
void launchTraceClosest(const LaunchCtx& c, int cur)
{
  if(c.wide)
    launchTraceClosestT<true>(c, cur);
  else
    launchTraceClosestT<false>(c, cur);
}
void launchShade(const LaunchCtx& c, int cur, bool first)
{
  dim3 grid(c.persistentBlocks), block(SHADE_BLOCK);
  if(c.visualization)
  {
#define MI_LAUNCH_SHADE_VIZ(S, F) \
  hipLaunchKernelGGL((k_shade_viz<S, F>), grid, block, 0, c.stream, c.sceneDev, c.fcDev, c.paths, c.queues, cur, (S ? 0 : c.sortMode), c.stats)
    if(c.simpleMaterials)
    {
      if(first) MI_LAUNCH_SHADE_VIZ(true, true); else MI_LAUNCH_SHADE_VIZ(true, false);
    }
    else
    {
      if(first) MI_LAUNCH_SHADE_VIZ(false, true); else MI_LAUNCH_SHADE_VIZ(false, false);
    }
#undef MI_LAUNCH_SHADE_VIZ
    return;
  }
#define MI_LAUNCH_SHADE(C, S, F) \
  hipLaunchKernelGGL((k_shade<C, S, F>), grid, block, 0, c.stream, c.sceneDev, c.fcDev, c.paths, c.queues, cur, (S ? 0 : c.sortMode), c.stats)
#define MI_LAUNCH_SHADE_F(C, S) do { if(first) MI_LAUNCH_SHADE(C, S, true); else MI_LAUNCH_SHADE(C, S, false); } while(0)
  if(c.simpleMaterials)
  {
    if(c.collectCounters) MI_LAUNCH_SHADE_F(true, true); else MI_LAUNCH_SHADE_F(false, true);
  }
  else
  {
    if(c.collectCounters) MI_LAUNCH_SHADE_F(true, false); else MI_LAUNCH_SHADE_F(false, false);
  }
#undef MI_LAUNCH_SHADE_F
#undef MI_LAUNCH_SHADE
}
void launchTraceShadow(const LaunchCtx& c, int nxt)
{
  if(c.wide)
    launchTraceShadowT<true>(c, nxt);
  else
    launchTraceShadowT<false>(c, nxt);
}
void launchFlushSurvivors(const LaunchCtx& c, int cur)
{
  hipLaunchKernelGGL(k_flush_survivors, dim3(c.persistentBlocks), dim3(256), 0, c.stream, c.paths, c.queues, cur);
}
void launchFinishSample(const LaunchCtx& c, int sampleIndex, float4* accum, float* depth, float4* albedo, float4* normal)
{
  unsigned grid = (unsigned(c.fc.numSlots) + 255u) / 256u;
  hipLaunchKernelGGL(k_finish_sample, dim3(grid), dim3(256), 0, c.stream, c.fc, c.sceneDev, c.fcDev, c.paths, c.ownedTiles, sampleIndex, accum, depth, albedo, normal);
}
void launchSelection(const LaunchCtx& c, uint32_t* selection)
{
  unsigned grid = (unsigned(c.fc.numSlots) + SEL_BLOCK - 1) / SEL_BLOCK;
  if(c.wide)
    hipLaunchKernelGGL(k_selection<true>, dim3(grid), dim3(SEL_BLOCK), 0, c.stream, c.scene, c.fc, c.ownedTiles, selection);
  else
    hipLaunchKernelGGL(k_selection<false>, dim3(grid), dim3(SEL_BLOCK), 0, c.stream, c.scene, c.fc, c.ownedTiles, selection);
}

}
```

### vk_gltf_renderer_amd/csrc/device/pt_shade_body.h

```cpp
  const DevScene&    sc = uniformConst(*scp);
  const FrameConsts& fc = uniformConst(*fcp);
  const bool         stateInQueue = fc.stateInQueue != 0;
  __shared__ uint32_t s_prefix[NSUB + 1];
  __shared__ uint32_t s_push[4];
  __shared__ float    s_srgb[256];
#ifndef SHADE_NO_DEFERRED_MISS
  constexpr bool DEFER_MISS = !FIRST;
#else
  constexpr bool DEFER_MISS = false;
#endif
  __shared__ uint32_t s_missPos[DEFER_MISS ? 2 * SHADE_BLOCK : 1];
  __shared__ uint32_t s_missCount;
  const bool          deferMiss = DEFER_MISS && !hasFlag(fc.frameInfo.flags, MI_SCENE_USE_INFINITE_PLANE) && !hasFlag(fc.frameInfo.flags, MI_SCENE_USE_HDR_ENVIRONMENT);
  if(threadIdx.x == 0)
    s_missCount = 0;
  auto finishMisses = [&](bool all) {
    __syncthreads();
    const uint32_t n = s_missCount;
    if(n == 0u || (!all && n < uint32_t(SHADE_BLOCK)))
      return;
    const uint32_t take = min(n, uint32_t(SHADE_BLOCK)), base = n - take;
    uint32_t       pos = 0;
    if(threadIdx.x < take)
      pos = s_missPos[base + threadIdx.x];
    __syncthreads();
    if(threadIdx.x == 0)
      s_missCount = base;
    if(threadIdx.x < take)
    {
      const uint32_t slot  = Q.active[cur].slot[pos];
      const float4   d4    = Q.active[cur].dir[pos];
      const float4   misc4 = stateInQueue ? Q.active[cur].misc[pos] : P.misc[slot];
      const float4   tp4   = stateInQueue ? Q.active[cur].aux2[pos] : P.throughput[slot];
      const float4   rad4  = stateInQueue ? Q.active[cur].rad[pos] : P.radiance[slot];
      f3             radiance = xyz(rad4);
      f3             envColor;
      float          mis;
      missEnvironment(sc, fc, xyz(d4), tp4.w, envColor, mis);
      radiance += xyz(tp4) * mis * envColor;
      uint32_t flags = __float_as_uint(misc4.y) & (PF_INSIDE | PF_NOT_SOLID | (0xffu << PF_DEPTH_SHIFT) | (0xffu << PF_SCATTER_SHIFT));
      if(SIMPLE)
        flags &= ~uint32_t(PF_INSIDE);
      const bool solid = !(flags & PF_NOT_SOLID);
      P.radiance[slot] = make_float4(radiance.x, radiance.y, radiance.z, __uint_as_float(__float_as_uint(fmaxf(fabsf(rad4.w), 0.0f)) | (solid ? 0u : RADW_NOT_SOLID)));
      if(P.misc)
        P.misc[slot] = make_float4(misc4.x, __uint_as_float(flags), misc4.z, misc4.w);
    }
    __syncthreads();
  };
  constexpr bool CAN_SORT = !SIMPLE;
  __shared__ uint32_t s_order[CAN_SORT ? SORT_WINDOW : 1];
  __shared__ uint16_t s_segCount[CAN_SORT ? SORT_SEGMENTS : 1][SORT_BINS];
  __shared__ uint32_t s_binBase[SORT_BINS + 1];
  static_assert(SHADE_BLOCK == 256, "one table entry per thread");
  if(blockIdx.x == 0 && threadIdx.x < 8)
  {
    Q.counters[QC_HEADS_TRACE + threadIdx.x] = 0;
    Q.counters[QC_HEADS_SHADOW + threadIdx.x]   = 0;
    Q.counters[QC_HEADS_OVERFLOW + threadIdx.x] = 0;
    if(threadIdx.x == 0)
      Q.counters[QC_CAND_POOL] = Q.counters[QC_RESOLVE] = Q.counters[QC_OVERFLOW] = 0;
  }
  queuePrefix(&Q.counters[cur ? QC_PAIR1 : QC_PAIR0], s_prefix);
  const uint32_t count      = s_prefix[NSUB];
  const int      nxt        = cur ^ 1;
  constexpr uint32_t ROUNDS = CAN_SORT ? SORT_ROUNDS : 1u;
  constexpr uint32_t WINDOW = ROUNDS * SHADE_BLOCK;
  const uint32_t     numWindows = (count + WINDOW - 1) / WINDOW;
  if(blockIdx.x >= numWindows)
    return;
  s_srgb[threadIdx.x] = sc.srgbLut[threadIdx.x];
  __syncthreads();
  const uint32_t wave = threadIdx.x >> 6, lane = threadIdx.x & 63u;
  for(uint32_t win = blockIdx.x; win < numWindows; win += gridDim.x)
  {
    uint32_t live = min(WINDOW, count - win * WINDOW);
    if(CAN_SORT && sortMode != 0)
    {
    uint32_t myPos[SORT_ROUNDS], myBin[SORT_ROUNDS], myRank[SORT_ROUNDS];
    for(uint32_t t = threadIdx.x; t < SORT_SEGMENTS * SORT_BINS; t += SHADE_BLOCK)
      (&s_segCount[0][0])[t] = 0;
    __syncthreads();
#pragma unroll
    for(uint32_t k = 0; k < SORT_ROUNDS; ++k)
    {
      const uint32_t i = win * WINDOW + k * SHADE_BLOCK + threadIdx.x;
      uint32_t       bin = SORT_BIN_DEAD;
      myPos[k]           = 0u;
      if(i < count)
      {
        myPos[k]            = queuePos(Q.subCap, s_prefix, i);
        const uint32_t slot = Q.active[cur].slot[myPos[k]];
        if(slot != QUEUE_DEAD)
        {
          const int tri = __float_as_int(Q.active[cur].aux[myPos[k]].y);
          if(tri < 0)
            bin = SORT_BIN_MISS;
          else
            bin = sortMode >= 2 ? uint32_t(sc.shadeTris[tri].materialID) % SORT_BIN_MISS : 0u;
        }
      }
      myBin[k] = bin;
      uint32_t           rank = 0;
      unsigned long long todo = __ballot(bin != SORT_BIN_DEAD);
      while(todo != 0ull)
      {
        const uint32_t           b = uint32_t(__builtin_amdgcn_readlane(int(bin), __ffsll((long long)todo) - 1));
        const unsigned long long m = __ballot(bin == b);
        if(bin == b)
          rank = laneCountBelow(m);
        if(lane == 0)
          s_segCount[k * 4 + wave][b] = uint16_t(__popcll(m));
        todo &= ~m;
      }
      myRank[k] = rank;
    }
    __syncthreads();
    if(threadIdx.x < SORT_BINS)
    {
      uint32_t acc = 0;
      for(uint32_t sgm = 0; sgm < SORT_SEGMENTS; ++sgm)
      {
        const uint32_t c = s_segCount[sgm][threadIdx.x];
        s_segCount[sgm][threadIdx.x] = uint16_t(acc);
        acc += c;
      }
      uint32_t incl = acc;
#pragma unroll
      for(int d = 1; d < SORT_BINS; d <<= 1)
      {
        const uint32_t t = uint32_t(__shfl_up(int(incl), d));
        if(threadIdx.x >= uint32_t(d))
          incl += t;
      }
      s_binBase[threadIdx.x] = incl - acc;
      if(threadIdx.x == SORT_BINS - 1)
        s_binBase[SORT_BINS] = incl;
    }
    __syncthreads();
#pragma unroll
    for(uint32_t k = 0; k < SORT_ROUNDS; ++k)
      if(myBin[k] != SORT_BIN_DEAD)
        s_order[s_binBase[myBin[k]] + s_segCount[k * 4 + wave][myBin[k]] + myRank[k]] = myPos[k];
    __syncthreads();
    live = s_binBase[SORT_BINS];
    }
   for(uint32_t round = 0; round * SHADE_BLOCK < live; ++round)
   {
    const uint32_t chunk   = win * ROUNDS + round;
    const uint32_t e       = round * SHADE_BLOCK + threadIdx.x;
    const bool     inRange = e < live;
    const uint32_t inPos   = !inRange ? 0u : ((CAN_SORT && sortMode != 0) ? s_order[e] : queuePos(Q.subCap, s_prefix, win * WINDOW + e));
    uint32_t       slot    = inRange ? Q.active[cur].slot[inPos] : QUEUE_DEAD;
    bool           alive = false, pushShadow = false;
// ... 95 lines not shown
        SPROF_END(6);
      }
      else if(hitT == INFINITE_F)
      {
        SPROF_BEGIN();
        bool backplate = false;
        if(firstRay)
        {
          solid             = false;
          if(needFirstHit)
            P.firstHit[pathSlotPixel(fc, slot)] = make_float4(rayDir.x, rayDir.y, rayDir.z, 0.0f);
          backplate = primaryMissBackplate(sc, fc, rayDir, radiance);
        }
        if(!backplate)
        {
          f3    envColor;
          float mis;
          missEnvironment(sc, fc, rayDir, lastSamplePdf, envColor, mis);
          radiance += throughput * mis * envColor;
        }
        done = true;
        SPROF_END(6);
      }

      if(!done)
      {
        PbrMaterial pbrMat;
        float worldFoot = (coneWidth + fc.pc.pixelAngle * hitT) / fmaxf(fabsf(dot(hit.geonrm, -rayDir)), 1e-3f);
        bool  unlit     = false;
        bool  catcherPlane = false;
        if(hitInfinitePlane)
        {
          pbrMat           = defaultPbrMaterial();
          pbrMat.baseColor = mk3(fc.frameInfo.infinitePlaneBaseColor);
          pbrMat.metallic  = fc.frameInfo.infinitePlaneMetallic;
          float r          = fc.frameInfo.infinitePlaneRoughness;
          pbrMat.roughness = mk2(r * r, r * r);
          pbrMat.N = hit.nrm; pbrMat.Ng = hit.nrm; pbrMat.Nc = hit.nrm;
          pbrMat.T = hit.tangent; pbrMat.B = hit.bitangent;
          if(hasFlag(fc.frameInfo.flags, MI_SCENE_INFINITE_PLANE_SHADOW_CATCHER))
          {
            catcherPlane = true;
            coneWidth    = worldFoot;
            if(FIRST && needFirstHit)
              P.firstHit[pathSlotPixel(fc, slot)] = make_float4(1e34f, 1e34f, 1e34f, __uint_as_float(TEMPORAL_ID_INVALID));
            DirectLight dl;
            sampleLights(sc, fc, hit.pos, seed, dl);
            const bool traceIt = dot(dl.direction, hit.nrm) > 0.0f && dl.pdf != 0.0f;
            f3         envColor;
            float      envPdf;
            sampleEnvironment(sc, fc, rayDir, envColor, envPdf);
            const float mis         = computeEnvHitMisWeight(sc, fc, lastSamplePdf, envPdf);
            const f3    unshadowed  = throughput * mis * envColor;
            if(!traceIt)
            {
              radiance += unshadowed;
              done = true;
            }
            else
            {
              shOrg = make_float4(hit.pos.x, hit.pos.y, hit.pos.z, INFINITE_F);
              shDir = make_float4(dl.direction.x, dl.direction.y, dl.direction.z, __uint_as_float(2u));
              shCon = make_float4(envColor.x, envColor.y, envColor.z, __uint_as_float(seed));
              shCon2     = make_float4(unshadowed.x, unshadowed.y, unshadowed.z, 0.0f);
              pushShadow = true;
              catcher    = true;
              float      r1 = rnd(seed), r2 = rnd(seed), r3 = rnd(seed);
              BsdfSample sd = bsdfSampleSimple(-rayDir, mk3(r1, r2, r3), pbrMat);
              if(sd.event_type == BSDF_EVENT_ABSORB)
                done = true;
              else
              {
                f3 offsetDir = dot(sd.k2, hit.geonrm) > 0.0f ? hit.geonrm : -hit.geonrm;
                rayOrigin    = safeOffsetRay(hit.pos, offsetDir);
                rayDir       = normalize(sd.k2);
                throughput *= sd.bsdf_over_pdf;
                lastSamplePdf = sd.pdf;
              }
            }
          }
        }
        else
        {
          const MiGltfShadeMaterial& mat = gat(sc.materials, materialID);
          MeshState                  mesh;
          mesh.N = hit.nrm; mesh.T = hit.tangent; mesh.B = hit.bitangent; mesh.Ng = hit.geonrm;
          mesh.tc0 = hit.uv0; mesh.tc1 = hit.uv1;
          mesh.isInside           = isInside;
          mesh.texGrad            = worldFoot * hit.texelDensity * fc.pc.texGradScale;
          mesh.baseColorVertexMul = hit.color;
          mesh.tex                = TexCtx{sc.texRefs, sc.texels, s_srgb, sc.texQuads};
          mesh.core0              = core0;
          SPROF_BEGIN();
          pbrMat                  = evaluateMaterial<SIMPLE, !FIRST>(sc, mat, mesh, taps);
          unlit                   = mat.unlit > 0;
          SPROF_END(1);
        }
        if(!catcherPlane)
        {
          if(firstRay)
          {
            if(needFirstHit)
              P.firstHit[pathSlotPixel(fc, slot)] = make_float4(hit.pos.x, hit.pos.y, hit.pos.z, __uint_as_float(hitInfinitePlane ? 0u : uint32_t(rnodeID + 1)));
            if(P.guideAlbedo)
            {
              float4 ga = make_float4(0, 0, 0, 0), gn = ga;
              if(fc.pc.numSamples > 1)
              {
                ga = P.guideAlbedo[slot];
                gn = P.guideNormal[slot];
              }
              guideWritten        = true;
              P.guideAlbedo[slot] = make_float4(ga.x + pbrMat.baseColor.x, ga.y + pbrMat.baseColor.y, ga.z + pbrMat.baseColor.z, ga.w + 1.0f);
              P.guideNormal[slot] = make_float4(gn.x + pbrMat.N.x, gn.y + pbrMat.N.y, gn.z + pbrMat.N.z, 0.0f);
            }
          }
          maxRoughness     = mk2(fmaxf(pbrMat.roughness.x, maxRoughness.x), fmaxf(pbrMat.roughness.y, maxRoughness.y));
          pbrMat.roughness = maxRoughness;
          if constexpr(VIZ)
          {
            f3        vizColour;
            const int vr = applyVisualization(pbrMat, hit, frontFace, fc.frameInfo.visualization, rprimID, primitiveID, ommState, vizColour);
            if(vr == VIZ_COLOR_OVERRIDE && firstRay)
            {
              radiance = vizColour;
              done     = true;
            }
          }
          if(!VIZ || !done)
          {
            radiance += pbrMat.emissive * throughput;
            if(unlit)
            {
              radiance += pbrMat.baseColor;
              done = true;
            }
          }

          bool volumeContinue = false;
          if(!SIMPLE && !done && isInside)
          {
            f3    ext, scat;
            float aniso;
            unpackMedium(P.medium[slot], ext, scat, aniso);
            if(maxComp(ext) > 0.0f || maxComp(scat) > 0.0f)
            {
              bool  scattered  = false;
              float maxScatter = maxComp(scat);
              f3    wiBefore = rayDir, originBefore = rayOrigin;
              if(maxScatter > VOLUME_MIN_SCATTER)
              {
                float maxExt      = maxComp(ext);
                float scatterDist = -logf(fmaxf(rnd(seed), VOLUME_RAND_FLOOR)) / maxExt;
                if(scatterDist < hitT)
                {
                  throughput *= mk3(1.0f) - (ext - scat) / maxExt;
                  rayOrigin     = rayOrigin + rayDir * scatterDist;
                  float r1 = rnd(seed), r2 = rnd(seed);
                  rayDir        = sampleHenyeyGreenstein(mk2(r1, r2), aniso, wiBefore);
                  lastSamplePdf = henyeyGreensteinPdf(dot(wiBefore, rayDir), aniso);
                  scattered     = true;
                }
                else
                  throughput *= exp3((mk3(maxExt) - ext) * hitT);
              }
              else
                throughput *= exp3(ext * (-hitT));
              if(scattered)
              {
                scatterBounces = min(scatterBounces + 1, 255);
                coneWidth += fc.pc.pixelAngle * length(rayOrigin - originBefore);
                DirectLight dl;
                sampleLights(sc, fc, rayOrigin, seed, dl);
                if(dl.pdf > 0.0f)
                {
                  float phasePdf = henyeyGreensteinPdf(dot(wiBefore, dl.direction), aniso);
                  float mis      = dl.pdf / (dl.pdf + phasePdf);
// ... 187 lines not shown
```

### vk_gltf_renderer_amd/csrc/device/pt_shading.h

```cpp
#pragma once
#include <cstddef>

#include "pt_light.h"

namespace pt {

constexpr float MIN_TRANSMISSION                = 0.01f;
constexpr float ANTIALIASING_STANDARD_DEVIATION = 0.4246609f;
constexpr int   RR_MIN_DEPTH                    = 3;
constexpr float VOLUME_MIN_SCATTER              = 0.001f;
constexpr float VOLUME_RAND_FLOOR               = 1.0e-10f;
constexpr int   VOLUME_FREE_BUDGET              = 64;
constexpr float RR_PCONT_FLOOR                  = 0.001f;
constexpr float RR_PCONT_CAP                    = 0.95f;
constexpr float MICROFACET_MIN_ROUGHNESS        = 0.0014142f;

PT_DEV bool hasFlag(int flags, int f) { return (flags & f) != 0; }

struct u3
{
  uint32_t x, y, z;
};
PT_DEV u3 getTriangleIndices(const DevPrim& rp, int prim)
{
// ... 27 lines not shown
  f4    color;
  f3    geonrm, shadowPos;
  f2    uv0, uv1;
  f3    tangent, bitangent;
  float texelDensity;
};
PT_DEV f3 pointOffset(f3 p, f3 p0, f3 p1, f3 p2, f3 n0, f3 n1, f3 n2, f3 bary)
{
  f3    tmpu = p - p0, tmpv = p - p1, tmpw = p - p2;
  float dotu = fminf(0.0f, dot(tmpu, n0)), dotv = fminf(0.0f, dot(tmpv, n1)), dotw = fminf(0.0f, dot(tmpw, n2));
  tmpu -= n0 * dotu;
  tmpv -= n1 * dotv;
  tmpw -= n2 * dotw;
  return p + tmpu * bary.x + tmpv * bary.y + tmpw * bary.z;
}
PT_DEV HitState getHitState(const float4* V0, const float4* V1, const float4* V2, uint32_t attrs, const DevPrim* rp, u3 ti, f3 bary, const float* w2o,
                            const float* o2w, f3 worldRayDir, bool* frontFaceOut = nullptr)
{
  HitState hit;
  const float4 a0 = V0[0], a1 = V0[1], a2 = V0[2], b0 = V1[0], b1 = V1[1], b2 = V1[2], c0 = V2[0], c1 = V2[1], c2 = V2[2];
  f3 pos0 = mk3(a0.x, a0.y, a0.z), pos1 = mk3(b0.x, b0.y, b0.z), pos2 = mk3(c0.x, c0.y, c0.z);
  f3 position  = pos0 * bary.x + pos1 * bary.y + pos2 * bary.z;
  hit.pos      = mulPoint(o2w, position);
  f3 geoNormal = normalize(cross(pos1 - pos0, pos2 - pos0));
  hit.geonrm   = normalize(mulTransposed(w2o, geoNormal));
  f3 nrm0 = geoNormal, nrm1 = geoNormal, nrm2 = geoNormal, normal = geoNormal;
  if(attrs & SHADE_HAS_NORMALS)
  {
    nrm0   = mk3(a0.w, a1.x, a1.y);
    nrm1   = mk3(b0.w, b1.x, b1.y);
    nrm2   = mk3(c0.w, c1.x, c1.y);
    normal = nrm0 * bary.x + nrm1 * bary.y + nrm2 * bary.z;
  }
  hit.nrm         = normalize(mulTransposed(w2o, normal));
  bool  frontFace = dot(hit.geonrm, worldRayDir) < 0.0f;
  if(frontFaceOut)
    *frontFaceOut = frontFace;
  float sideFlip  = frontFace ? 1.0f : -1.0f;
  f3    shadowPos = pointOffset(position, pos0, pos1, pos2, nrm0 * sideFlip, nrm1 * sideFlip, nrm2 * sideFlip, bary);
  hit.shadowPos   = mulPoint(o2w, shadowPos);
  hit.uv0 = (attrs & SHADE_HAS_UV0) ? mk2(a1.z, a1.w) * bary.x + mk2(b1.z, b1.w) * bary.y + mk2(c1.z, c1.w) * bary.z : mk2(0.0f, 0.0f);
  hit.uv1 = (attrs & SHADE_HAS_UV1) ? getInterpolatedVertexTexCoord(*rp, 1, ti, bary) : mk2(0.0f, 0.0f);
  if(attrs & SHADE_HAS_UV0)
  {
    const float2 a = make_float2(a1.z, a1.w), b = make_float2(b1.z, b1.w), c = make_float2(c1.z, c1.w);
    f3    we1 = mulVector(o2w, pos1 - pos0), we2 = mulVector(o2w, pos2 - pos0);
    float wArea = length(cross(we1, we2));
    f2    duv1 = mk2(b.x - a.x, b.y - a.y), duv2 = mk2(c.x - a.x, c.y - a.y);
    float uvArea     = fabsf(duv1.x * duv2.y - duv1.y * duv2.x);
    hit.texelDensity = sqrtf(fmaxf(uvArea, 1e-20f) / fmaxf(wArea, 1e-20f));
  }
  else
    hit.texelDensity = 0.0f;
  hit.color = (attrs & SHADE_HAS_COLORS) ? getInterpolatedVertexColor(*rp, ti, bary) : mk4(1.0f);
  f4 tng0, tng1, tng2;
  if(attrs & SHADE_HAS_TANGENTS)
  {
    tng0 = mk4(a2);
    tng1 = mk4(b2);
    tng2 = mk4(c2);
  }
  else
  {
    tng0 = tng1 = tng2 = makeFastTangent(normal);
  }
  hit.tangent   = normalize(xyz(tng0) * bary.x + xyz(tng1) * bary.y + xyz(tng2) * bary.z);
  hit.tangent   = mulVector(o2w, hit.tangent);
  hit.tangent   = normalize(hit.tangent - hit.nrm * dot(hit.nrm, hit.tangent));
  hit.bitangent = cross(hit.nrm, hit.tangent) * tng0.w;
  if(!frontFace)
    hit.geonrm = -hit.geonrm;
  if(dot(hit.geonrm, hit.nrm) < 0.0f)
  {
    hit.nrm       = -hit.nrm;
    hit.tangent   = -hit.tangent;
    hit.bitangent = -hit.bitangent;
  }
  f3 r = reflect(normalize(worldRayDir), hit.nrm);
  if(dot(r, hit.geonrm) < 0.0f)
    hit.nrm = hit.geonrm;
  return hit;
}

struct MeshState
{
  f3    N, T, B, Ng;
  f2    tc0, tc1;
  bool  isInside;
  float texGrad;
  f4    baseColorVertexMul;
  TexCtx tex;
  uint4 core0;
};
PT_DEV bool isTexturePresent(uint16_t t) { return t > 0; }
PT_DEV f4 fetchTexelRef(const TexCtx& tc, const DevTexRef& R, uint32_t levelOffset, int w, int x, int y)
{
  uchar4 p = gat(tc.texels, texelIndex(levelOffset, w, x, y));
  if(R.srgb)
    return mk4(tc.lut[p.x], tc.lut[p.y], tc.lut[p.z], float(p.w) * (1.0f / 255.0f));
  return mk4(float(p.x) * (1.0f / 255.0f), float(p.y) * (1.0f / 255.0f), float(p.z) * (1.0f / 255.0f), float(p.w) * (1.0f / 255.0f));
}
PT_DEV f4 decodeTexel(const TexCtx& tc, bool srgb, uint32_t p)
{
  const uint32_t r = p & 0xffu, g = (p >> 8) & 0xffu, b = (p >> 16) & 0xffu, a = p >> 24;
  if(srgb)
    return mk4(tc.lut[r], tc.lut[g], tc.lut[b], float(a) * (1.0f / 255.0f));
  return mk4(float(r) * (1.0f / 255.0f), float(g) * (1.0f / 255.0f), float(b) * (1.0f / 255.0f), float(a) * (1.0f / 255.0f));
}
PT_DEV f4 decodeTexelRef(const TexCtx& tc, const DevTexRef& R, uint32_t p) { return decodeTexel(tc, R.srgb != 0, p); }
PT_DEV f4 bilinearBlend(f4 a, f4 b, f4 c, f4 d, float tx, float ty)
{
#pragma clang fp contract(off)
  const float ux = 1.0f - tx, uy = 1.0f - ty;
  auto        ch = [&](float p00, float p10, float p01, float p11) { return __fmaf_rn(__fmaf_rn(p11, tx, p01 * ux), ty, __fmaf_rn(p10, tx, p00 * ux) * uy); };
  return mk4(ch(a.x, b.x, c.x, d.x), ch(a.y, b.y, c.y, d.y), ch(a.z, b.z, c.z, d.z), ch(a.w, b.w, c.w, d.w));
}
PT_DEV f4 levelBlend(f4 a, f4 b, float f)
{
#pragma clang fp contract(off)
  const float u = 1.0f - f;
  return mk4(__fmaf_rn(b.x, f, a.x * u), __fmaf_rn(b.y, f, a.y * u), __fmaf_rn(b.z, f, a.z * u), __fmaf_rn(b.w, f, a.w * u));
}
struct QuadTap
{
  uint32_t index;
  float    tx, ty;
  bool     dupX, dupY;
};
PT_DEV bool hasQuadPath(const TexCtx& tc, const DevTexRef& R) { return tc.quads && R.wrapS != MI_WRAP_MIRRORED_REPEAT && R.wrapT != MI_WRAP_MIRRORED_REPEAT; }
PT_DEV uint32_t levelOffsetWH(uint32_t level0, int W, int H, int level)
{
  uint32_t off = level0;
  for(int l = 0; l < level; ++l)
    off += uint32_t(max(1, W >> l)) * uint32_t(max(1, H >> l));
  return off;
}
PT_DEV uint32_t levelOffsetRef(const DevTexRef& R, int level) { return levelOffsetWH(R.level0, int(R.width), int(R.height), level); }
PT_DEV void bilinearCoords(f2 uv, int w, int h, int& ix, int& iy, float& tx, float& ty)
{
#pragma clang fp contract(off)
  float fx = uv.x * float(w), fy = uv.y * float(h);
  fx -= 0.5f;
  fy -= 0.5f;
  const float flx = floorf(fx), fly = floorf(fy);
  ix = int(flx);
  iy = int(fly);
  tx = fx - flx;
  ty = fy - fly;
}
PT_DEV QuadTap quadTapWH(int W, int H, int wrapS, int wrapT, f2 uv, int level, uint32_t off)
{
  const int      w = max(1, W >> level), h = max(1, H >> level);
  int            ix, iy;
  QuadTap        t;
  bilinearCoords(uv, w, h, ix, iy, t.tx, t.ty);
  t.index = texelIndex(off, w, wrapCoord(ix, w, wrapS), wrapCoord(iy, h, wrapT));
  t.dupX  = wrapS == MI_WRAP_CLAMP_TO_EDGE && ix < 0;
  t.dupY  = wrapT == MI_WRAP_CLAMP_TO_EDGE && iy < 0;
  return t;
}
PT_DEV QuadTap quadTap(const DevTexRef& R, f2 uv, int level, uint32_t off) { return quadTapWH(int(R.width), int(R.height), R.wrapS, R.wrapT, uv, level, off); }
PT_DEV f4 quadFilterS(const TexCtx& tc, bool srgb, float tx, float ty, bool dupX, bool dupY, const uint4 q)
{
  const f4 a = decodeTexel(tc, srgb, q.x), b = decodeTexel(tc, srgb, dupX ? q.x : q.y);
  const f4 c = decodeTexel(tc, srgb, dupY ? q.x : q.z), d = decodeTexel(tc, srgb, dupY ? (dupX ? q.x : q.y) : (dupX ? q.z : q.w));
  return bilinearBlend(a, b, c, d, tx, ty);
}
PT_DEV f4 quadFilter(const TexCtx& tc, const DevTexRef& R, const QuadTap& t, const uint4 q) { return quadFilterS(tc, R.srgb != 0, t.tx, t.ty, t.dupX, t.dupY, q); }
PT_DEV f4 sampleLevelRef(const TexCtx& tc, const DevTexRef& R, f2 uv, int level, int filter)
{
  if(filter != MI_FILTER_NEAREST && hasQuadPath(tc, R))
  {
    const QuadTap t = quadTap(R, uv, level, levelOffsetRef(R, level));
    return quadFilter(tc, R, t, gat(tc.quads, t.index));
  }
  const uint32_t off = levelOffsetRef(R, level);
  int   w = max(1, int(R.width) >> level), h = max(1, int(R.height) >> level);
  if(filter == MI_FILTER_NEAREST)
  {
    const float fx = uv.x * float(w), fy = uv.y * float(h);
    return fetchTexelRef(tc, R, off, w, wrapCoord(int(floorf(fx)), w, R.wrapS), wrapCoord(int(floorf(fy)), h, R.wrapT));
  }
  int   ix, iy, x0, x1, y0, y1;
  float tx, ty;
  bilinearCoords(uv, w, h, ix, iy, tx, ty);
  wrapCoordPair(ix, w, R.wrapS, x0, x1);
  wrapCoordPair(iy, h, R.wrapT, y0, y1);
  const uint32_t* T   = reinterpret_cast<const uint32_t*>(tc.texels);
  const uint32_t  p00 = gat(T, texelIndex(off, w, x0, y0)), p10 = gat(T, texelIndex(off, w, x1, y0));
  const uint32_t  p01 = gat(T, texelIndex(off, w, x0, y1)), p11 = gat(T, texelIndex(off, w, x1, y1));
  f4    a = decodeTexelRef(tc, R, p00), b = decodeTexelRef(tc, R, p10);
  f4    c = decodeTexelRef(tc, R, p01), d = decodeTexelRef(tc, R, p11);
  return bilinearBlend(a, b, c, d, tx, ty);
}
PT_DEV f2 texUv(const float* U, f2 t)
{
#pragma clang fp contract(off)
  return mk2(__fmaf_rn(t.y, U[2], t.x * U[0]) + U[4], __fmaf_rn(t.y, U[3], t.x * U[1]) + U[5]);
}
PT_DEV float texLodOf(float rx2, float ry2)
{
  const float rho = sqrtf(fmaxf(rx2, ry2));
  return rho > 0.0f ? log2f(rho) : -126.0f;
}
PT_DEV float texLod(const float* U, float texGrad, float W, float H)
{
#pragma clang fp contract(off)
  const float ax = (U[0] * texGrad) * W, bx = (U[1] * texGrad) * H, ay = (U[2] * texGrad) * W, by = (U[3] * texGrad) * H;
  return texLodOf(__fmaf_rn(bx, bx, ax * ax), __fmaf_rn(by, by, ay * ay));
}
PT_DEV float texLodIdentity(float texGrad, float W, float H)
{
#pragma clang fp contract(off)
  const float ax = texGrad * W, by = texGrad * H;
  return texLodOf(ax * ax, by * by);
}
PT_DEV DevTexRef loadTexRef(const DevTexRef* refs, uint32_t slot)
{
#if !defined(__HIPCC__)
  return refs[slot];
#else
  typedef uint32_t u32x4 __attribute__((ext_vector_type(4)));
  typedef uint32_t u32x3 __attribute__((ext_vector_type(3)));
  const DevTexRef* p = refs + slot;
  u32x4            a, b;
  u32x3            c;
  asm volatile("global_load_dwordx4 %0, %3, off\n\tglobal_load_dwordx4 %1, %3, off offset:16\n\tglobal_load_dwordx3 %2, %3, off offset:32\n\ts_waitcnt vmcnt(0)"
               : "=&v"(a), "=&v"(b), "=&v"(c)
               : "v"(p)
               : "memory");
  DevTexRef R;
  uint32_t* W = reinterpret_cast<uint32_t*>(&R);
  W[0] = a[0]; W[1] = a[1]; W[2] = a[2]; W[3] = a[3]; W[4] = b[0]; W[5] = b[1]; W[6] = b[2]; W[7] = b[3]; W[8] = c[0]; W[9] = c[1]; W[10] = c[2];
  return R;
#endif
}
__device__ __noinline__ f4 getTextureRef(TexCtx tc, uint32_t slot, f2 tc0, f2 tc1, float texGrad)
{
#ifdef MI_PT_DIAG_NO_TEX
  return mk4(0.5f + 1e-3f * (tc0.x + tc1.y + texGrad + float(slot)));
#endif
  const DevTexRef R  = loadTexRef(tc.refs, slot);
  f2              t  = R.texCoord == 0 ? tc0 : tc1;
  const float*    U  = R.uv;
  f2              uv = texUv(U, t);
  if(R.width == 0)
    return mk4(1.0f);
  float lod = 0.0f;
  if(texGrad > 0.0f)
    lod = texLod(U, texGrad, float(R.width), float(R.height));
  if(lod <= 0.0f)
    return sampleLevelRef(tc, R, uv, 0, R.magFilter);
  float maxLevel = float(int(R.numLevels) - 1);
  lod            = fminf(lod, maxLevel);
  if(R.mipmapMode == MI_FILTER_NEAREST)
    return sampleLevelRef(tc, R, uv, min(int(floorf(lod + 0.5f)), int(R.numLevels) - 1), R.minFilter);
  int   l0 = int(floorf(lod)), l1 = min(l0 + 1, int(R.numLevels) - 1);
  float f  = lod - float(l0);
  if(R.minFilter != MI_FILTER_NEAREST && hasQuadPath(tc, R) && !(f == 0.0f || l1 == l0))
  {
    const uint32_t off0 = levelOffsetRef(R, l0), off1 = off0 + uint32_t(max(1, int(R.width) >> l0)) * uint32_t(max(1, int(R.height) >> l0));
    const QuadTap  t0 = quadTap(R, uv, l0, off0), t1 = quadTap(R, uv, l1, off1);
    const uint4   q0 = gat(tc.quads, t0.index), q1 = gat(tc.quads, t1.index);
    const f4      a = quadFilter(tc, R, t0, q0), b = quadFilter(tc, R, t1, q1);
    return levelBlend(a, b, f);
  }
  f4    a  = sampleLevelRef(tc, R, uv, l0, R.minFilter);
  if(f == 0.0f || l1 == l0)
    return a;
  f4 b = sampleLevelRef(tc, R, uv, l1, R.minFilter);
  return levelBlend(a, b, f);
}
#ifndef MI_PT_CORE_TEX_BATCH
#define MI_PT_CORE_TEX_BATCH 1
#endif
struct CoreTap
{
  uint32_t i0, i1;
  float    tx0, ty0, tx1, ty1, f;
  uint32_t bits;
};
enum : uint32_t { CP_FAST = 1u, CP_TWO = 2u, CP_SRGB = 4u, CP_DUPX0 = 8u, CP_DUPY0 = 16u, CP_DUPX1 = 32u, CP_DUPY1 = 64u, CP_SLOW = 128u };
PT_DEV CoreTap coreTexPlan(const TexCtx& tc, const uint4 c, f2 tc0, f2 tc1, float texGrad)
{
  CoreTap p;
  p.i0 = p.i1 = 0u;
  p.tx0 = p.ty0 = p.tx1 = p.ty1 = p.f = 0.0f;
  p.bits = 0u;
  const int W = int(c.y & 0xffffu), H = int(c.y >> 16);
  if(W == 0)
    return p;
#ifdef MI_PT_DIAG_NO_TEX
  p.bits = CP_SLOW;
  return p;
#endif
  if(!(c.z & CT_FAST) || !tc.quads)
  {
    p.bits = CP_SLOW;
    return p;
  }
  const f2 t   = (c.z & CT_TEXCOORD1) ? tc1 : tc0;
  f2       uv  = t;
  float    lod = 0.0f;
  if(c.z & CT_TRANSFORM)
  {
    const float* U6 = gat(tc.refs, c.w).uv;
    const float  U[6] = {U6[0], U6[1], U6[2], U6[3], U6[4], U6[5]};
    uv = texUv(U, t);
    if(texGrad > 0.0f)
      lod = texLod(U, texGrad, float(W), float(H));
  }
  else if(texGrad > 0.0f)
    lod = texLodIdentity(texGrad, float(W), float(H));
  const int wrapS = int((c.z >> CT_WRAPS_SHIFT) & 3u), wrapT = int((c.z >> CT_WRAPT_SHIFT) & 3u), levels = int((c.z >> CT_LEVELS_SHIFT) & 0xffu);
  int   l0  = 0;
  bool  two = false;
  float f   = 0.0f;
  if(!(lod <= 0.0f))
  {
    lod = fminf(lod, float(levels - 1));
    if(!(c.z & CT_MIP_LINEAR))
      l0 = min(int(floorf(lod + 0.5f)), levels - 1);
    else
    {
      l0           = int(floorf(lod));
      const int l1 = min(l0 + 1, levels - 1);
      f            = lod - float(l0);
      two          = !(f == 0.0f || l1 == l0);
    }
  }
  const uint32_t off0 = levelOffsetWH(c.x, W, H, l0);
  const QuadTap  t0   = quadTapWH(W, H, wrapS, wrapT, uv, l0, off0);
  p.i0 = t0.index; p.tx0 = t0.tx; p.ty0 = t0.ty;
  p.bits = CP_FAST | ((c.z & CT_SRGB) ? CP_SRGB : 0u) | (t0.dupX ? CP_DUPX0 : 0u) | (t0.dupY ? CP_DUPY0 : 0u);
  if(two)
  {
    const uint32_t off1 = off0 + uint32_t(max(1, W >> l0)) * uint32_t(max(1, H >> l0));
    const QuadTap  t1   = quadTapWH(W, H, wrapS, wrapT, uv, l0 + 1, off1);
    p.i1 = t1.index; p.tx1 = t1.tx; p.ty1 = t1.ty; p.f = f;
    p.bits |= CP_TWO | (t1.dupX ? CP_DUPX1 : 0u) | (t1.dupY ? CP_DUPY1 : 0u);
  }
  return p;
}
PT_DEV void coreTexIssue(const TexCtx& tc, const CoreTap& p, uint4& q0, uint4& q1)
{
  q0 = q1 = make_uint4(0u, 0u, 0u, 0u);
  if(p.bits & CP_FAST)
  {
    q0 = gat(tc.quads, p.i0);
    if(p.bits & CP_TWO)
      q1 = gat(tc.quads, p.i1);
  }
}
PT_DEV f4 coreTexFinish(const TexCtx& tc, const CoreTap& p, const uint4& q0, const uint4& q1, uint32_t slot, f2 tc0, f2 tc1, float texGrad)
{
  if(p.bits & CP_SLOW)
    return getTextureRef(tc, slot, tc0, tc1, texGrad);
  if(!(p.bits & CP_FAST))
    return mk4(1.0f);
  const bool srgb = (p.bits & CP_SRGB) != 0u;
  const f4   a    = quadFilterS(tc, srgb, p.tx0, p.ty0, (p.bits & CP_DUPX0) != 0u, (p.bits & CP_DUPY0) != 0u, q0);
  if(!(p.bits & CP_TWO))
    return a;
  const f4 b = quadFilterS(tc, srgb, p.tx1, p.ty1, (p.bits & CP_DUPX1) != 0u, (p.bits & CP_DUPY1) != 0u, q1);
  return levelBlend(a, b, p.f);
}
PT_DEV f3 multiToSingleScatterAlbedo(f3 rho)
{
  f3 t = mk3(4.09712f) + rho * 4.20863f - sqrt3(mk3(9.59217f) + rho * 41.6808f + rho * rho * 17.7126f);
  return mk3(1.0f) - t * t;
}
PT_DEV f3 convertSGToMR(f3 diffuseColor, f3 specularColor, float glossiness, float& metallic, f2& roughness)
{
  const float dielectricSpecular = 0.04f;
  float       specularIntensity  = fmaxf(specularColor.x, fmaxf(specularColor.y, specularColor.z));
  metallic                       = smoothstepf(dielectricSpecular + 0.01f, dielectricSpecular + 0.05f, specularIntensity);
  f3 baseColor;
  if(metallic > 0.0f)
    baseColor = specularColor;
  else
  {
    baseColor = diffuseColor / (1.0f - dielectricSpecular * (1.0f - metallic));
    baseColor = clamp3(baseColor, 0.0f, 1.0f);
  }
  float r   = 1.0f - glossiness;
  roughness = mk2(r * r, r * r);
  return baseColor;
}
template <bool SIMPLE, bool CORE = false>
PT_DEV PbrMaterial evaluateMaterial(const DevScene& sc, const MiGltfShadeMaterial& m, const MeshState& st, unsigned& taps)
{
#define TEX(slot) (++taps, getTextureRef(st.tex, slot, st.tc0, st.tc1, st.texGrad))
  PbrMaterial p = defaultPbrMaterial();
  static_assert(offsetof(MiGltfShadeMaterial, pbrBaseColorTexture) % 8 == 0 && offsetof(MiGltfShadeMaterial, occlusionTexture) == offsetof(MiGltfShadeMaterial, pbrBaseColorTexture) + 8,
                "core texture slots: base colour, normal, metallic-roughness, emissive, occlusion");
  const uint32_t* slotWords = reinterpret_cast<const uint32_t*>(&m.pbrBaseColorTexture);
  const uint32_t  sw0 = slotWords[0], sw1 = slotWords[1], sw2 = slotWords[2];
  const uint16_t  texBaseColor = uint16_t(sw0 & 0xffffu), texNormal = uint16_t(sw0 >> 16), texMetallicRoughness = uint16_t(sw1 & 0xffffu),
                 texEmissive = uint16_t(sw1 >> 16), texOcclusion = uint16_t(sw2 & 0xffffu);
  CoreTap cp0{};
  uint4   cq0 = make_uint4(0u, 0u, 0u, 0u), cq1 = cq0;
  if(CORE && MI_PT_CORE_TEX_BATCH)
  {
    const bool  present = m.pbrModel != MI_PBR_SPECULAR_GLOSSINESS && isTexturePresent(texBaseColor);
    const uint4 c       = st.core0;
    cp0                 = coreTexPlan(st.tex, present ? c : make_uint4(0u, 0u, 0u, 0u), st.tc0, st.tc1, st.texGrad);
    coreTexIssue(st.tex, cp0, cq0, cq1);
  }
  if(m.pbrModel == MI_PBR_SPECULAR_GLOSSINESS)
  {
    f4    diffuse    = mk4(m.pbrDiffuseFactor[0], m.pbrDiffuseFactor[1], m.pbrDiffuseFactor[2], m.pbrDiffuseFactor[3]) * st.baseColorVertexMul;
    float glossiness = m.pbrGlossinessFactor;
    f3    specular   = mk3(m.pbrSpecularFactor);
    if(isTexturePresent(m.pbrDiffuseTexture))
      diffuse *= TEX(m.pbrDiffuseTexture);
    if(isTexturePresent(m.pbrSpecularGlossinessTexture))
    {
      f4 s = TEX(m.pbrSpecularGlossinessTexture);
      specular *= xyz(s);
      glossiness *= s.w;
    }
    p.baseColor = convertSGToMR(xyz(diffuse), specular, glossiness, p.metallic, p.roughness);
    p.opacity   = diffuse.w;
  }
  else
  {
    f4 baseColor = mk4(m.pbrBaseColorFactor[0], m.pbrBaseColorFactor[1], m.pbrBaseColorFactor[2], m.pbrBaseColorFactor[3]) * st.baseColorVertexMul;
    if(isTexturePresent(texBaseColor))
      baseColor *= (CORE && MI_PT_CORE_TEX_BATCH) ? (++taps, coreTexFinish(st.tex, cp0, cq0, cq1, texBaseColor, st.tc0, st.tc1, st.texGrad)) : TEX(texBaseColor);
    p.baseColor     = xyz(baseColor);
    p.opacity       = baseColor.w;
    float roughness = m.pbrRoughnessFactor, metallic = m.pbrMetallicFactor;
    if(isTexturePresent(texMetallicRoughness))
    {
      f4 s = TEX(texMetallicRoughness);
      roughness *= s.y;
      metallic *= s.z;
    }
    roughness   = fmaxf(roughness, MICROFACET_MIN_ROUGHNESS);
    p.roughness = mk2(roughness * roughness, roughness * roughness);
    p.metallic  = clampf(metallic, 0.0f, 1.0f);
  }
  p.occlusion = m.occlusionStrength;
  if(isTexturePresent(texOcclusion))
  {
    float occ   = TEX(texOcclusion).x;
    p.occlusion = 1.0f + p.occlusion * (occ - 1.0f);
  }
  p.N  = st.N;
  p.T  = st.T;
  p.B  = st.B;
  p.Ng = st.Ng;
  bool needsTangentUpdate = false;
  if(isTexturePresent(texNormal))
  {
    f3 nv = xyz(TEX(texNormal));
    nv    = nv * 2.0f - mk3(1.0f);
    nv *= mk3(m.normalTextureScale, m.normalTextureScale, 1.0f);
    p.N                = normalize(st.T * nv.x + st.B * nv.y + st.N * nv.z);
    needsTangentUpdate = true;
  }
  p.emissive = mk3(m.emissiveFactor);
  if(isTexturePresent(texEmissive))
    p.emissive *= xyz(TEX(texEmissive));
  p.emissive            = max3(mk3(0.0f), p.emissive);
  if(!SIMPLE)
  {
    p.attenuationColor    = mk3(m.attenuationColor);
    p.attenuationDistance = m.attenuationDistance;
    p.thickness           = m.thicknessFactor;
    if(isTexturePresent(m.thicknessTexture))
      p.thickness *= TEX(m.thicknessTexture).y;
  }
  p.specularColor = mk3(m.specularColorFactor);
  if(isTexturePresent(m.specularColorTexture))
    p.specularColor *= xyz(TEX(m.specularColorTexture));
  p.specular = m.specularFactor;
  if(isTexturePresent(m.specularTexture))
    p.specular *= TEX(m.specularTexture).w;
  float ior1 = 1.0f, ior2 = m.ior;
  if(!SIMPLE && st.isInside && (p.thickness > 0.0f))
  {
    ior1 = ior2;
    ior2 = 1.0f;
  }
  p.ior1         = ior1;
  p.ior2         = ior2;
  bool needsTangentUpdateAniso = false;
  if(!SIMPLE)
  {
  p.transmission = m.transmissionFactor;
  if(isTexturePresent(m.transmissionTexture))
    p.transmission *= TEX(m.transmissionTexture).x;
  f3 ms = mk3(m.multiscatterColorFactor);
  if(ms.x > 0.0f || ms.y > 0.0f || ms.z > 0.0f)
  {
    f3 ssa               = multiToSingleScatterAlbedo(ms);
    f3 attC              = -log3(max3(p.attenuationColor, mk3(0.001f))) / fmaxf(p.attenuationDistance, 0.001f);
    p.scatterCoefficient = attC * ssa;
  }
  p.scatterAnisotropy  = m.scatterAnisotropy;
  p.clearcoat          = m.clearcoatFactor;
  p.clearcoatRoughness = m.clearcoatRoughness;
  p.Nc                 = p.N;
  if(isTexturePresent(m.clearcoatTexture))
    p.clearcoat *= TEX(m.clearcoatTexture).x;
  if(isTexturePresent(m.clearcoatRoughnessTexture))
    p.clearcoatRoughness *= TEX(m.clearcoatRoughnessTexture).y;
  if(isTexturePresent(m.clearcoatNormalTexture))
  {
    f3 nv = xyz(TEX(m.clearcoatNormalTexture));
    nv    = nv * 2.0f - mk3(1.0f);
    p.Nc  = normalize(p.T * nv.x + p.B * nv.y + p.Nc * nv.z);
  }
  p.clearcoatRoughness = fmaxf(p.clearcoatRoughness, 0.001f);
  float iridescence = m.iridescenceFactor, iridescenceThickness = m.iridescenceThicknessMaximum;
  p.iridescenceIor = m.iridescenceIor;
  if(isTexturePresent(m.iridescenceTexture))
    iridescence *= TEX(m.iridescenceTexture).x;
  if(isTexturePresent(m.iridescenceThicknessTexture))
  {
    float t              = TEX(m.iridescenceThicknessTexture).y;
    iridescenceThickness = lerpf(m.iridescenceThicknessMinimum, m.iridescenceThicknessMaximum, t);
  }
  p.iridescence          = (iridescenceThickness > 0.0f) ? iridescence : 0.0f;
  p.iridescenceThickness = iridescenceThickness;
  float anisotropyStrength = m.anisotropyStrength;
  if(anisotropyStrength > 0.0f)
  {
    f2 dir = mk2(1.0f, 0.0f);
    if(isTexturePresent(m.anisotropyTexture))
    {
      f4 a = TEX(m.anisotropyTexture);
      dir  = normalize(mk2(a.x, a.y) * 2.0f - mk2(1.0f, 1.0f));
      anisotropyStrength *= a.z;
    }
    p.roughness.x = lerpf(p.roughness.y, 1.0f, anisotropyStrength * anisotropyStrength);
    float s = m.anisotropyRotation[0], c = m.anisotropyRotation[1];
    dir                = mk2(c * dir.x + s * dir.y, c * dir.y - s * dir.x);
    p.T                = p.T * dir.x + p.B * dir.y;
    needsTangentUpdateAniso = true;
  }
  }
  needsTangentUpdate = needsTangentUpdate || needsTangentUpdateAniso;
  if(needsTangentUpdate)
  {
    p.B         = normalize(cross(p.N, p.T));
    float bsign = signfz(dot(st.B, p.B));
    p.B         = p.B * bsign;
    p.T         = normalize(cross(p.B, p.N) * bsign);
  }
  if(!SIMPLE)
  {
  p.sheenColor = mk3(m.sheenColorFactor);
  if(isTexturePresent(m.sheenColorTexture))
    p.sheenColor *= xyz(TEX(m.sheenColorTexture));
  p.sheenRoughness = m.sheenRoughnessFactor;
  if(isTexturePresent(m.sheenRoughnessTexture))
    p.sheenRoughness *= TEX(m.sheenRoughnessTexture).w;
  p.sheenRoughness            = fmaxf(MICROFACET_MIN_ROUGHNESS, p.sheenRoughness);
  p.dispersion                = m.dispersion;
  p.diffuseTransmissionFactor = m.diffuseTransmissionFactor;
  if(isTexturePresent(m.diffuseTransmissionTexture))
    p.diffuseTransmissionFactor *= TEX(m.diffuseTransmissionTexture).w;
  p.diffuseTransmissionColor = mk3(m.diffuseTransmissionColor);
  if(isTexturePresent(m.diffuseTransmissionColorTexture))
    p.diffuseTransmissionColor *= xyz(TEX(m.diffuseTransmissionColorTexture));
  p.retroreflection = m.retroreflectionFactor;
  if(isTexturePresent(m.retroreflectionTexture))
    p.retroreflection *= TEX(m.retroreflectionTexture).x;
  }
#undef TEX
  return p;
}

PT_DEV f3 safeOffsetRay(f3 p, f3 dir)
{
  const float scaleValue = 256.0f;
  int         ix = int(scaleValue * dir.x), iy = int(scaleValue * dir.y), iz = int(scaleValue * dir.z);
  f3 op = mk3(__int_as_float(__float_as_int(p.x) + ((p.x < 0) ? -ix : ix)), __int_as_float(__float_as_int(p.y) + ((p.y < 0) ? -iy : iy)),
              __int_as_float(__float_as_int(p.z) + ((p.z < 0) ? -iz : iz)));
  const float origin = 1.0f / 32.0f, floatScale = 1.0f / 65536.0f;
  return mk3(fabsf(p.x) < origin ? p.x + floatScale * dir.x : op.x, fabsf(p.y) < origin ? p.y + floatScale * dir.y : op.y,
             fabsf(p.z) < origin ? p.z + floatScale * dir.z : op.z);
}

PT_DEV float getOpacityFast(const DevScene& sc, int triIndex, f3 bary)
{
  const DevAlphaTri rec  = sc.alphaTris[triIndex];
  const uint32_t    flg  = rec.c.z;
  const uint32_t    mode = flg & AT_MODE_MASK;
  if(mode == MI_ALPHA_OPAQUE)
    return 1.0f;
  float alpha = rec.b.z;
  if(flg & AT_HAS_TEXTURE)
  {
    f2          uv = mk2(rec.a.x, rec.a.y) * bary.x + mk2(rec.a.z, rec.a.w) * bary.y + mk2(rec.b.x, rec.b.y) * bary.z;
    const int   w = int(rec.c.y & 0xffffu), h = int(rec.c.y >> 16);
    const int   wrapS = int((flg >> AT_WRAPS_SHIFT) & 3u), wrapT = int((flg >> AT_WRAPT_SHIFT) & 3u);
    const uchar4* texels = sc.texels + rec.c.x;
    float       fx = uv.x * float(w), fy = uv.y * float(h);
    float       ta;
    if(!(flg & AT_LINEAR))
      ta = float(texels[texelIndex(0u, w, wrapCoord(int(floorf(fx)), w, wrapS), wrapCoord(int(floorf(fy)), h, wrapT))].w) * (1.0f / 255.0f);
    else
    {
      fx -= 0.5f;
      fy -= 0.5f;
      float flx = floorf(fx), fly = floorf(fy);
      float tx = fx - flx, ty = fy - fly;
      float a, b, c, d;
      if(sc.texQuads && wrapS != MI_WRAP_MIRRORED_REPEAT && wrapT != MI_WRAP_MIRRORED_REPEAT)
      {
        const int   ix = int(flx), iy = int(fly);
        const uint4 q  = sc.texQuads[rec.c.x + texelIndex(0u, w, wrapCoord(ix, w, wrapS), wrapCoord(iy, h, wrapT))];
        const bool  dupX = wrapS == MI_WRAP_CLAMP_TO_EDGE && ix < 0, dupY = wrapT == MI_WRAP_CLAMP_TO_EDGE && iy < 0;
        a = float(q.x >> 24) * (1.0f / 255.0f);
        b = float((dupX ? q.x : q.y) >> 24) * (1.0f / 255.0f);
        c = float((dupY ? q.x : q.z) >> 24) * (1.0f / 255.0f);
        d = float((dupY ? (dupX ? q.x : q.y) : (dupX ? q.z : q.w)) >> 24) * (1.0f / 255.0f);
      }
      else
      {
        int x0, x1, y0, y1;
        wrapCoordPair(int(flx), w, wrapS, x0, x1);
        wrapCoordPair(int(fly), h, wrapT, y0, y1);
        a = float(texels[texelIndex(0u, w, x0, y0)].w) * (1.0f / 255.0f); b = float(texels[texelIndex(0u, w, x1, y0)].w) * (1.0f / 255.0f);
        c = float(texels[texelIndex(0u, w, x0, y1)].w) * (1.0f / 255.0f); d = float(texels[texelIndex(0u, w, x1, y1)].w) * (1.0f / 255.0f);
      }
      ta = (a * (1.0f - tx) + b * tx) * (1.0f - ty) + (c * (1.0f - tx) + d * tx) * ty;
    }
    alpha *= ta;
  }
  if(flg & AT_HAS_COLORS)
  {
    const uint32_t v = rec.c.w;
    alpha *= (float(v & 0xffu) / 255.0f) * bary.x + (float((v >> 8) & 0xffu) / 255.0f) * bary.y + (float((v >> 16) & 0xffu) / 255.0f) * bary.z;
  }
  if(mode == MI_ALPHA_MASK)
    return alpha >= rec.b.w ? 1.0f : 0.0f;
  return alpha;
}
PT_DEV int32_t shadeRecordMaterial(const MiGltfRenderNode& rn)
{
  return max(0, rn.materialID);
}
PT_DEV DevShadeTri makeShadeRecord(const DevScene& sc, const DevTri& T)
{
// ... 301 lines not shown
```

### vk_gltf_renderer_amd/pathtracer.py

```python
import ctypes as C

import numpy as np

from . import _capi as capi


HIT_DTYPE = np.dtype([("t", "<f4"), ("b1", "<f4"), ("b2", "<f4"), ("flags", "<u4"), ("renderNode", "<i4"), ("renderPrimID", "<i4"), ("triangle", "<u4"),
                      ("materialID", "<i4"), ("position", "<f4", (3,)), ("reserved0", "<f4"), ("normal", "<f4", (3,)), ("reserved1", "<f4")])
assert HIT_DTYPE.itemsize == 64
_QUERY_MODES = {"closest": capi.MI_PT_QUERY_CLOSEST, "any": capi.MI_PT_QUERY_ANY, "nearest_k": capi.MI_PT_QUERY_NEAREST_K}
_QUERY_ALPHA = {"opaque": capi.MI_PT_QUERY_ALPHA_OPAQUE, "cutoff": capi.MI_PT_QUERY_ALPHA_CUTOFF, "stochastic": capi.MI_PT_QUERY_ALPHA_STOCHASTIC}
_QUERY_CULL = {"none": capi.MI_PT_QUERY_CULL_NONE, "material": capi.MI_PT_QUERY_CULL_MATERIAL}


class MiError(RuntimeError):
    pass


def _check_host(rc):
    if rc != 0:
        raise MiError(f"libmi_host: rc={rc}: {capi.host_lib().mi_host_last_error().decode()}")


def _check_pt(rc):
# ... 188 lines not shown

    def update_materials(self, materials, num_materials, texture_infos, num_texture_infos):
        _check_pt(self._l.mi_pt_update_materials(self._p, materials, int(num_materials), texture_infos, int(num_texture_infos)))

    def set_deformation(self, scene):
        d = scene.deformation if scene is not None else None
        _check_pt(self._l.mi_pt_set_deformation(self._p, C.byref(d) if d is not None else None))
        self._deforming = d is not None

    def update_deformation(self, joint_matrices, morph_weights, defer_build=False):
        def keep(a):
            return a if a is None or isinstance(a, C._Pointer) else np.ascontiguousarray(a, dtype=np.float32)

        def ptr(a):
            return a if a is None or isinstance(a, C._Pointer) else a.ctypes.data_as(C.POINTER(C.c_float))
        jm, mw = keep(joint_matrices), keep(morph_weights)
        _check_pt(self._l.mi_pt_update_deformation(self._p, ptr(jm), ptr(mw), capi.MI_PT_DEFORM_DEFER_BUILD if defer_build else 0))

    def set_vertex_updates(self, prims, recompute_normals=False):
        ids = [int(p) for p in (prims if prims is not None else [])]
        arr = (C.c_int32 * max(len(ids), 1))(*ids)
        _check_pt(self._l.mi_pt_set_vertex_updates(self._p, arr, len(ids), capi.MI_PT_VERTICES_RECOMPUTE_NORMALS if recompute_normals else 0))

    def update_vertices(self, updates, defer_build=False):
        def is_device(a):
            return hasattr(a, "data_ptr") and hasattr(a, "is_contiguous")
        table = (capi.MiPtVertexUpdate * max(len(updates), 1))()
        keep, forms = [], set()
        for k, (prim, streams) in enumerate(updates.items()):
            streams = tuple(streams) if isinstance(streams, (tuple, list)) else (streams,)
            if not 1 <= len(streams) <= 3 or streams[0] is None:
                raise ValueError(f"update_vertices: primitive {prim}: positions, or (positions, normals, tangents)")
            streams = streams + (None,) * (3 - len(streams))
            u = table[k]
            u.renderPrimID = int(prim)
            for name, a, width in zip(("positions", "normals", "tangents"), streams, (3, 3, 4)):
                if a is None:
                    continue
                forms.add(is_device(a))
                if is_device(a):
                    if str(a.dtype) != "torch.float32" or not a.is_contiguous() or a.device.type != "cuda":
                        raise ValueError(f"update_vertices: primitive {prim}: {name} must be a contiguous float32 tensor on the device")
                    count, ptr = a.numel(), a.data_ptr()
                else:
                    a = np.ascontiguousarray(a, dtype=np.float32)
                    count, ptr = a.size, a.ctypes.data
                keep.append(a)
                if count % width:
                    raise ValueError(f"update_vertices: primitive {prim}: {name} holds {count} floats, no multiple of {width}")
                if name == "positions":
                    u.vertexCount = count // width
                elif count // width != u.vertexCount:
                    raise ValueError(f"update_vertices: primitive {prim}: {name} has {count // width} vertices, positions {u.vertexCount}")
                setattr(u, name, ptr)
        if len(forms) > 1:
            raise ValueError("update_vertices: numpy arrays and device tensors in one call")
        fn = self._l.mi_pt_update_vertices_device if True in forms else self._l.mi_pt_update_vertices
        _check_pt(fn(self._p, table, len(updates), capi.MI_PT_DEFORM_DEFER_BUILD if defer_build else 0))

    def vertex_update_info(self):
        a = capi.MiPtVertexUpdateInfo()
        _check_pt(self._l.mi_pt_get_vertex_update_info(self._p, C.byref(a)))
        return {n: int(getattr(a, n)) for n, _ in a._fields_}

    ACCEL_MODES = {"rebuild": 0, "refit": 1, "auto": 2}

    def set_accel_update(self, mode, rebuild_cost_ratio=1.5):
        m = self.ACCEL_MODES[mode] if isinstance(mode, str) else int(mode)
        _check_pt(self._l.mi_pt_set_accel_update(self._p, m, C.c_float(rebuild_cost_ratio)))

    def accel_info(self):
        a = capi.MiPtAccelInfo()
        _check_pt(self._l.mi_pt_get_accel_info(self._p, C.byref(a)))
        return {n: getattr(a, n) for n, _ in a._fields_ if n != "reserved"}

    def set_accel_resident(self, enable=True):
        _check_pt(self._l.mi_pt_set_accel_resident(self._p, 1 if enable else 0))

    def accel_resident_info(self):
        a = capi.MiPtAccelResidentInfo()
        _check_pt(self._l.mi_pt_get_accel_resident_info(self._p, C.byref(a)))
        return {n: getattr(a, n) for n, _ in a._fields_}

    def read_vertices(self, prim):
        p = self._scene.desc.contents.renderPrimitives[prim]
        n = int(p.vertexCount)
        pos = np.zeros((n, 3), np.float32)
        nrm = np.zeros((n, 3), np.float32) if p.normals else None
        tan = np.zeros((n, 4), np.float32) if p.tangents else None
        f = lambda a: a.ctypes.data_as(C.POINTER(C.c_float)) if a is not None else None
        _check_pt(self._l.mi_pt_read_vertices(self._p, int(prim), f(pos), f(nrm), f(tan)))
        return pos, nrm, tan

    def update_from_scene(self, scene):
        d = scene.desc.contents
        deform = scene.deformation if getattr(self, "_deforming", False) else None
        if deform is not None:
            self.update_deformation(deform.jointMatrices, deform.morphWeights, defer_build=True)
        if scene.animation_changes & capi.MI_SCENE_CHANGED_MATERIALS:
            self.update_materials(d.materials, d.numMaterials, d.textureInfos, d.numTextureInfos)
        self.update_render_nodes(d.renderNodes, d.numRenderNodes, d.renderNodeVisible)
        self.update_lights(d.lights, d.numLights)

    def set_environment(self, hdr):
        _check_pt(self._l.mi_pt_set_environment(self._p, hdr.env if hdr is not None else None))

    def resize(self, width, height):
        _check_pt(self._l.mi_pt_resize(self._p, width, height))
        self.width, self.height = width, height

    def set_frame_info(self, fi):
        _check_pt(self._l.mi_pt_set_frame_info(self._p, C.byref(fi)))

    def set_sky(self, sky):
        _check_pt(self._l.mi_pt_set_sky(self._p, C.byref(sky)))

    def set_tile_partition(self, rank, world, tile_size=64):
        _check_pt(self._l.mi_pt_set_tile_partition(self._p, rank, world, tile_size))

    def bind_accum(self, device_ptr):
        _check_pt(self._l.mi_pt_bind_accum(self._p, C.c_void_p(device_ptr)))

    def bind_guides(self, albedo_ptr=0, normal_ptr=0, depth_ptr=0):
        _check_pt(self._l.mi_pt_bind_guides(self._p, C.c_void_p(albedo_ptr or None), C.c_void_p(normal_ptr or None), C.c_void_p(depth_ptr or None)))

    def set_frame_queue(self, depth):
        _check_pt(self._l.mi_pt_set_frame_queue(self._p, int(depth)))

    def render_frame(self, params, stream=None):
        _check_pt(self._l.mi_pt_render_frame(self._p, C.byref(params), C.c_void_p(stream or 0)))

    def render_frames(self, params, num_frames, stream=None):
        _check_pt(self._l.mi_pt_render_frames(self._p, C.byref(params), num_frames, C.c_void_p(stream or 0)))

    def synchronize(self):
        _check_pt(self._l.mi_pt_synchronize(self._p))

    def read_accum(self):
        out = np.empty((self.height, self.width, 4), dtype=np.float32)
        _check_pt(self._l.mi_pt_read_accum(self._p, out.ctypes.data_as(C.POINTER(C.c_float))))
        return out

    def write_accum(self, img):
        img = np.ascontiguousarray(img, dtype=np.float32)
        assert img.shape == (self.height, self.width, 4)
        _check_pt(self._l.mi_pt_write_accum(self._p, img.ctypes.data_as(C.POINTER(C.c_float))))

    def read_guides(self):
        a = np.empty((self.height, self.width, 4), dtype=np.float32)
        n = np.empty((self.height, self.width, 4), dtype=np.float32)
        _check_pt(self._l.mi_pt_read_guides(self._p, a.ctypes.data_as(C.POINTER(C.c_float)), n.ctypes.data_as(C.POINTER(C.c_float))))
        return a, n

    def read_selection(self):
        out = np.empty((self.height, self.width), dtype=np.uint32)
        _check_pt(self._l.mi_pt_read_selection(self._p, out.ctypes.data_as(C.POINTER(C.c_uint32))))
        return out

    def set_camera_rays(self, rays, unit=False):
        flags = capi.MI_PT_CAMERA_RAYS_UNIT if unit else 0
        if rays is None:
            _check_pt(self._l.mi_pt_set_camera_rays(self._p, None, 0, 0))
            self._camera_rays = None
            return
        torch_form = type(rays).__module__.split(".")[0] == "torch"
        if not torch_form:
# ... 234 lines not shown
```

Baseline: 761.2.

## Stage material and texture-ref tables in LDS for simple-material shading

Adds a shade-kernel variant that copies the material table and texture-reference records into dynamic LDS at block start, then reads material fields and texture refs from LDS instead of global memory during material evaluation. A host-side plan checks the tables fit a 48 KiB budget and that occupancy holds at the target waves before enabling it. An environment switch defaults it on. It costs a per-block copy of up to 48 KiB and LDS pressure, and it only applies when the scene has simple materials.

```diff
diff --git a/include/mi_pt.h b/include/mi_pt.h
--- a/include/mi_pt.h
+++ b/include/mi_pt.h
@@ -198,6 +198,16 @@
   uint64_t materialPatches;
 } MiPtAccelResidentInfo;
 MI_PT_API int mi_pt_get_accel_resident_info(MiPt* pt, MiPtAccelResidentInfo* info);
+typedef struct MiPtShadeLdsInfo
+{
+  int32_t  mode;
+  int32_t  inUse;
+  uint32_t numMaterials;
+  uint32_t numTexRefs;
+  uint32_t bytes;
+  uint32_t reserved;
+} MiPtShadeLdsInfo;
+MI_PT_API int mi_pt_get_shade_lds_info(MiPt* pt, MiPtShadeLdsInfo* info);
 MI_PT_API int mi_pt_read_vertices(MiPt* pt, int renderPrimID, float* positions, float* normals, float* tangents);
 
 MI_PT_API int mi_pt_destroy(MiPt* pt);
diff --git a/vk_gltf_renderer_amd/_capi.py b/vk_gltf_renderer_amd/_capi.py
--- a/vk_gltf_renderer_amd/_capi.py
+++ b/vk_gltf_renderer_amd/_capi.py
@@ -149,6 +149,10 @@
                 ("visibilityRefits", C.c_uint64), ("materialPatches", C.c_uint64)]
 
 
+class MiPtShadeLdsInfo(C.Structure):
+    _fields_ = [("mode", i32), ("inUse", i32), ("numMaterials", C.c_uint32), ("numTexRefs", C.c_uint32), ("bytes", C.c_uint32), ("reserved", C.c_uint32)]
+
+
 class MiPtTemporalParams(C.Structure):
     _fields_ = [("iterations", i32), ("sigmaLuminance", f32), ("sigmaNormal", f32), ("sigmaDepth", f32), ("alpha", f32), ("momentsAlpha", f32),
                 ("maxHistory", f32), ("normalCos", f32), ("depthTolerance", f32)]
@@ -188,6 +192,7 @@
 assert C.sizeof(MiSceneFrameInfo) == 396
 assert C.sizeof(MiPtAccelInfo) == 64
 assert C.sizeof(MiPtAccelResidentInfo) == 40
+assert C.sizeof(MiPtShadeLdsInfo) == 24
 assert C.sizeof(MiPtRay) == 32
 assert C.sizeof(MiPtRayHit) == 64
 assert C.sizeof(MiPtQueryOptions) == 32
@@ -328,6 +333,7 @@
     "mi_pt_get_accel_info": (i32, [VP, P(MiPtAccelInfo)]),
     "mi_pt_set_accel_resident": (i32, [VP, i32]),
     "mi_pt_get_accel_resident_info": (i32, [VP, P(MiPtAccelResidentInfo)]),
+    "mi_pt_get_shade_lds_info": (i32, [VP, P(MiPtShadeLdsInfo)]),
     "mi_pt_read_first_hit": (i32, [VP, P(f32)]),
     "mi_pt_set_temporal": (i32, [VP, i32]),
     "mi_pt_read_motion": (i32, [VP, P(f32)]),
diff --git a/vk_gltf_renderer_amd/csrc/device/mi_pt_api.hip b/vk_gltf_renderer_amd/csrc/device/mi_pt_api.hip
--- a/vk_gltf_renderer_amd/csrc/device/mi_pt_api.hip
+++ b/vk_gltf_renderer_amd/csrc/device/mi_pt_api.hip
@@ -69,6 +69,7 @@
   bool   hostCollapse   = false;
   bool   coreTex        = true;
   bool   shadowDeposit  = true;
+  bool   shadeLds       = true;
   int    maxItersDiag   = 0;
   int    failBuildAt    = 0;
   bool   candPoolSet    = false;
@@ -105,6 +106,7 @@
     maxItersDiag   = num("MI_PT_DIAG_MAX_ITERS", 0);
     coreTex        = num("MI_PT_CORE_TEX", 1) != 0;
     shadowDeposit  = num("MI_PT_SHADOW_DEPOSIT", 1) != 0;
+    shadeLds       = num("MI_PT_SHADE_LDS", 1) != 0;
     failBuildAt    = num("MI_PT_DIAG_FAIL_BUILD", 0);
     if(const char* e = getenv("MI_PT_DIAG_CAND_POOL"))
     {
@@ -148,6 +150,9 @@
   bool                        wide      = true;
   pt::DevScene                scene{};
   bool                        hasAlpha = false, hasAlphaTest = false, hasVolumeScatter = false, simpleMaterials = true, hasTransmissive = false;
+  pt::ShadeLdsPlan            shadeLdsPlan{};
+  bool                        shadeLdsResident = false;
+  void planShadeLds() { shadeLdsPlan = shadeLdsResident ? pt::shadeLdsPlan(int(materials.count), int(texRefs.count)) : pt::ShadeLdsPlan{}; }
   static constexpr int        FC_RING = 32;
   DevBuf<pt::DevScene>        sceneDev;
   bool                        sceneDevDirty = true;
@@ -1363,6 +1368,8 @@
     deriveTextureRecords(pt.get(), sd->materials, sd->numMaterials, sd->textureInfos, sd->numTextureInfos, refs, core);
     HIP_TRY(pt->texRefs.upload(refs.data(), refs.size()));
     HIP_TRY(pt->coreTex.upload(core.data(), core.size()));
+    pt->shadeLdsResident = pt::shadeLdsStaysResident(pt::SHADE_LDS_BUDGET);
+    pt->planShadeLds();
   }
   {
     float lut[256];
@@ -1495,6 +1502,7 @@
       std::swap(pt->texRefs.ptr, drefs.ptr); std::swap(pt->texRefs.count, drefs.count);
       pt->scene.texInfos = pt->texInfos.ptr;
       pt->scene.texRefs  = pt->texRefs.ptr;
+      pt->planShadeLds();
     }
     else
     {
@@ -2066,6 +2074,19 @@
   return MI_PT_OK;
 }
 
+int mi_pt_get_shade_lds_info(MiPt* pt, MiPtShadeLdsInfo* out)
+{
+  if(!pt || !out)
+    return fail(MI_PT_ERR_ARGUMENT, "mi_pt_get_shade_lds_info: null argument");
+  memset(out, 0, sizeof(*out));
+  out->mode         = pt->shadeLdsPlan.mode;
+  out->inUse        = (pt->shadeLdsPlan.mode != pt::SHADE_LDS_NONE && pt->sw.shadeLds && pt->simpleMaterials) ? 1 : 0;
+  out->numMaterials = pt->shadeLdsPlan.numMaterials;
+  out->numTexRefs   = pt->shadeLdsPlan.numTexRefs;
+  out->bytes        = pt->shadeLdsPlan.bytes;
+  return MI_PT_OK;
+}
+
 int mi_pt_read_vertices(MiPt* pt, int renderPrimID, float* positions, float* normals, float* tangents)
 {
   FLUSH_PENDING(pt);
@@ -2340,6 +2361,8 @@
   c.wide             = pt->wide;
   c.collectCounters  = pt->collectCounters;
   c.shadowDeposit    = pt->sw.shadowDeposit;
+  c.shadeLds         = pt->sw.shadeLds;
+  c.shadeLdsPlan     = pt->shadeLdsPlan;
   {
     c.sortMode = pt->sw.sortMode;
   }
diff --git a/vk_gltf_renderer_amd/csrc/device/pt_kernels.h b/vk_gltf_renderer_amd/csrc/device/pt_kernels.h
--- a/vk_gltf_renderer_amd/csrc/device/pt_kernels.h
+++ b/vk_gltf_renderer_amd/csrc/device/pt_kernels.h
@@ -2,6 +2,7 @@
 #include <hip/hip_runtime.h>
 
 #include "pt_scene.h"
+#include "pt_shade_lds_plan.h"
 #include "pt_temporal.h"
 
 namespace pt {
@@ -27,7 +28,10 @@
   bool            shadowDeposit;
   int             sortMode;
   bool            visualization;
+  bool            shadeLds;
+  ShadeLdsPlan    shadeLdsPlan;
 };
+bool shadeLdsStaysResident(uint32_t dynamicLdsBytes);
 
 void launchBuildShadeRecords(const DevScene& scene, uint32_t numTris, DevShadeTri* out, hipStream_t s);
 void launchBuildAlphaRecords(const DevScene& scene, uint32_t numTris, DevAlphaTri* out, hipStream_t s);
diff --git a/vk_gltf_renderer_amd/csrc/device/pt_kernels.hip b/vk_gltf_renderer_amd/csrc/device/pt_kernels.hip
--- a/vk_gltf_renderer_amd/csrc/device/pt_kernels.hip
+++ b/vk_gltf_renderer_amd/csrc/device/pt_kernels.hip
@@ -1196,6 +1196,17 @@
 {
   constexpr bool COUNT = false, VIZ = true;
 #include "pt_shade_body.h"
+}
+static_assert(sizeof(MiGltfShadeMaterial) == SHADE_LDS_MATERIAL_BYTES && sizeof(MiGltfShadeMaterial) % 16 == 0 && sizeof(DevTexRef) == SHADE_LDS_TEXREF_BYTES,
+              "pt_shade_lds_plan.h sizes the tables");
+template <bool COUNT, bool FIRST>
+__global__ void __launch_bounds__(SHADE_BLOCK, SHADE_SIMPLE_WAVES) k_shade_lds(const DevScene* __restrict__ scp, const FrameConsts* __restrict__ fcp, PathSoA P, Queues Q, int cur, int sortMode, StatCounters* stats,
+                                                                            uint32_t ldsMaterials, uint32_t ldsTexRefs)
+{
+  constexpr bool SIMPLE = true, VIZ = false;
+#define SHADE_BODY_LDS_TABLES
+#include "pt_shade_body.h"
+#undef SHADE_BODY_LDS_TABLES
 }
 
 template <int MODE>
@@ -2210,6 +2221,22 @@
 #undef MI_LAUNCH_SHADE_VIZ
     return;
   }
+  if(c.simpleMaterials && c.shadeLds && c.shadeLdsPlan.mode != SHADE_LDS_NONE)
+  {
+#define MI_LAUNCH_SHADE_LDS(C, F)                                                                                                                        \
+  hipLaunchKernelGGL((k_shade_lds<C, F>), grid, block, c.shadeLdsPlan.bytes, c.stream, c.sceneDev, c.fcDev, c.paths, c.queues, cur, 0, c.stats, \
+                     c.shadeLdsPlan.numMaterials, c.shadeLdsPlan.numTexRefs)
+    if(c.collectCounters)
+    {
+      if(first) MI_LAUNCH_SHADE_LDS(true, true); else MI_LAUNCH_SHADE_LDS(true, false);
+    }
+    else
+    {
+      if(first) MI_LAUNCH_SHADE_LDS(false, true); else MI_LAUNCH_SHADE_LDS(false, false);
+    }
+#undef MI_LAUNCH_SHADE_LDS
+    return;
+  }
 #define MI_LAUNCH_SHADE(C, S, F) \
   hipLaunchKernelGGL((k_shade<C, S, F>), grid, block, 0, c.stream, c.sceneDev, c.fcDev, c.paths, c.queues, cur, (S ? 0 : c.sortMode), c.stats)
 #define MI_LAUNCH_SHADE_F(C, S) do { if(first) MI_LAUNCH_SHADE(C, S, true); else MI_LAUNCH_SHADE(C, S, false); } while(0)
@@ -2223,6 +2250,17 @@
   }
 #undef MI_LAUNCH_SHADE_F
 #undef MI_LAUNCH_SHADE
+}
+bool shadeLdsStaysResident(uint32_t dynamicLdsBytes)
+{
+  const void* kernels[4] = {(const void*)k_shade_lds<false, false>, (const void*)k_shade_lds<false, true>, (const void*)k_shade_lds<true, false>, (const void*)k_shade_lds<true, true>};
+  for(const void* k : kernels)
+  {
+    int blocks = 0;
+    if(hipOccupancyMaxActiveBlocksPerMultiprocessor(&blocks, k, SHADE_BLOCK, size_t(dynamicLdsBytes)) != hipSuccess || blocks < SHADE_SIMPLE_WAVES)
+      return false;
+  }
+  return true;
 }
 void launchTraceShadow(const LaunchCtx& c, int nxt)
 {
diff --git a/vk_gltf_renderer_amd/csrc/device/pt_shade_body.h b/vk_gltf_renderer_amd/csrc/device/pt_shade_body.h
--- a/vk_gltf_renderer_amd/csrc/device/pt_shade_body.h
+++ b/vk_gltf_renderer_amd/csrc/device/pt_shade_body.h
@@ -70,6 +70,38 @@
   if(blockIdx.x >= numWindows)
     return;
   s_srgb[threadIdx.x] = sc.srgbLut[threadIdx.x];
+#ifdef SHADE_BODY_LDS_TABLES
+  extern __shared__ uint4 s_tables[];
+  {
+    const uint32_t matQuads = shadeLdsMaterialBytes(ldsMaterials) / 16u, refWords = ldsTexRefs * uint32_t(sizeof(DevTexRef) / 4);
+    if constexpr(SHADE_LDS_MATERIAL_STRIDE == sizeof(MiGltfShadeMaterial))
+    {
+      const uint4* srcMat = reinterpret_cast<const uint4*>(sc.materials);
+      for(uint32_t i = threadIdx.x; i < matQuads; i += SHADE_BLOCK)
+        s_tables[i] = gat(srcMat, i);
+    }
+    else
+    {
+      constexpr uint32_t RECORD_WORDS = uint32_t(sizeof(MiGltfShadeMaterial) / 4);
+      uint32_t*          dstMat = reinterpret_cast<uint32_t*>(s_tables);
+      const uint32_t*    srcMat = reinterpret_cast<const uint32_t*>(sc.materials);
+      for(uint32_t i = threadIdx.x; i < ldsMaterials * RECORD_WORDS; i += SHADE_BLOCK)
+        dstMat[(i / RECORD_WORDS) * (SHADE_LDS_MATERIAL_STRIDE / 4u) + i % RECORD_WORDS] = gat(srcMat, i);
+    }
+    const uint4* srcRef = reinterpret_cast<const uint4*>(sc.texRefs);
+    for(uint32_t i = threadIdx.x; i < refWords / 4u; i += SHADE_BLOCK)
+      s_tables[matQuads + i] = gat(srcRef, i);
+    uint32_t*       dstWords = reinterpret_cast<uint32_t*>(s_tables + matQuads);
+    const uint32_t* srcWords = reinterpret_cast<const uint32_t*>(sc.texRefs);
+    for(uint32_t i = (refWords & ~3u) + threadIdx.x; i < refWords; i += SHADE_BLOCK)
+      dstWords[i] = gat(srcWords, i);
+  }
+  typedef const PT_LDS_AS MiGltfShadeMaterial* LdsMaterialPtr;
+  typedef const PT_LDS_AS DevTexRef*           LdsTexRefPtr;
+  typedef const PT_LDS_AS uint8_t*             LdsBytePtr;
+  const LdsBytePtr   ldsMaterialTable = (LdsBytePtr)(s_tables);
+  const LdsTexRefPtr ldsTexRefTable   = (LdsTexRefPtr)(ldsMaterialTable + shadeLdsMaterialBytes(ldsMaterials));
+#endif
   __syncthreads();
   const uint32_t wave = threadIdx.x >> 6, lane = threadIdx.x & 63u;
   for(uint32_t win = blockIdx.x; win < numWindows; win += gridDim.x)
@@ -331,7 +363,11 @@
         }
         else
         {
+#ifdef SHADE_BODY_LDS_TABLES
+          const PT_LDS_AS MiGltfShadeMaterial& mat = *(LdsMaterialPtr)(ldsMaterialTable + min(uint32_t(materialID), ldsMaterials - 1u) * SHADE_LDS_MATERIAL_STRIDE);
+#else
           const MiGltfShadeMaterial& mat = gat(sc.materials, materialID);
+#endif
           MeshState                  mesh;
           mesh.N = hit.nrm; mesh.T = hit.tangent; mesh.B = hit.bitangent; mesh.Ng = hit.geonrm;
           mesh.tc0 = hit.uv0; mesh.tc1 = hit.uv1;
@@ -341,7 +377,13 @@
           mesh.tex                = TexCtx{sc.texRefs, sc.texels, s_srgb, sc.texQuads};
           mesh.core0              = core0;
           SPROF_BEGIN();
+#ifdef SHADE_BODY_LDS_TABLES
+          mesh.refsLds            = ldsTexRefTable;
+          mesh.numRefsLds         = ldsTexRefs;
+          pbrMat                  = evaluateMaterial<SIMPLE, !FIRST, true>(sc, mat, mesh, taps);
+#else
           pbrMat                  = evaluateMaterial<SIMPLE, !FIRST>(sc, mat, mesh, taps);
+#endif
           unlit                   = mat.unlit > 0;
           SPROF_END(1);
         }
diff --git a/vk_gltf_renderer_amd/csrc/device/pt_shade_lds_plan.h b/vk_gltf_renderer_amd/csrc/device/pt_shade_lds_plan.h
--- /dev/null
+++ b/vk_gltf_renderer_amd/csrc/device/pt_shade_lds_plan.h
@@ -0,0 +1,53 @@
+#pragma once
+#include <cstdint>
+
+namespace pt {
+
+constexpr uint32_t SHADE_LDS_BUDGET         = 48u * 1024u;
+constexpr uint32_t SHADE_LDS_MATERIAL_BYTES = 288u;
+#ifndef MI_PT_SHADE_LDS_STRIDE
+#define MI_PT_SHADE_LDS_STRIDE 288
+#endif
+constexpr uint32_t SHADE_LDS_MATERIAL_STRIDE = MI_PT_SHADE_LDS_STRIDE;
+static_assert(SHADE_LDS_MATERIAL_STRIDE >= SHADE_LDS_MATERIAL_BYTES && SHADE_LDS_MATERIAL_STRIDE % 4 == 0, "a record every stride bytes, word aligned");
+constexpr uint32_t SHADE_LDS_TEXREF_BYTES   = 44u;
+
+enum ShadeLdsMode : int
+{
+  SHADE_LDS_NONE               = 0,
+  SHADE_LDS_MATERIALS          = 1,
+  SHADE_LDS_MATERIALS_AND_REFS = 2,
+};
+
+struct ShadeLdsPlan
+{
+  int      mode;
+  uint32_t numMaterials;
+  uint32_t numTexRefs;
+  uint32_t bytes;
+};
+
+constexpr uint32_t shadeLdsMaterialBytes(uint32_t numMaterials) { return (numMaterials * SHADE_LDS_MATERIAL_STRIDE + 15u) & ~15u; }
+
+inline ShadeLdsPlan shadeLdsPlan(int numMaterials, int numTextureInfos)
+{
+  ShadeLdsPlan p{SHADE_LDS_NONE, 0u, 0u, 0u};
+  if(numMaterials <= 0 || ((uint64_t(numMaterials) * SHADE_LDS_MATERIAL_STRIDE + 15u) & ~uint64_t(15u)) > SHADE_LDS_BUDGET)
+    return p;
+  p.mode         = SHADE_LDS_MATERIALS;
+  p.numMaterials = uint32_t(numMaterials);
+  p.bytes        = shadeLdsMaterialBytes(p.numMaterials);
+  if(numTextureInfos > 0)
+  {
+    const uint64_t both = (uint64_t(p.bytes) + uint64_t(numTextureInfos) * SHADE_LDS_TEXREF_BYTES + 15u) & ~uint64_t(15u);
+    if(both <= SHADE_LDS_BUDGET)
+    {
+      p.mode       = SHADE_LDS_MATERIALS_AND_REFS;
+      p.numTexRefs = uint32_t(numTextureInfos);
+      p.bytes      = uint32_t(both);
+    }
+  }
+  return p;
+}
+
+}
diff --git a/vk_gltf_renderer_amd/csrc/device/pt_shading.h b/vk_gltf_renderer_amd/csrc/device/pt_shading.h
--- a/vk_gltf_renderer_amd/csrc/device/pt_shading.h
+++ b/vk_gltf_renderer_amd/csrc/device/pt_shading.h
@@ -133,6 +133,17 @@
   return hit;
 }
 
+#if defined(__HIPCC__)
+#define PT_LDS_AS __attribute__((address_space(3)))
+#else
+#define PT_LDS_AS
+#endif
+template <class U, class T> struct PtrLike { typedef const U* type; };
+#if defined(__HIPCC__)
+template <class U, class T> struct PtrLike<U, PT_LDS_AS T> { typedef const PT_LDS_AS U* type; };
+template <class U, class T> struct PtrLike<U, const PT_LDS_AS T> { typedef const PT_LDS_AS U* type; };
+#endif
+template <class P> PT_DEV f3 mk3p(P p) { return f3{p[0], p[1], p[2]}; }
 struct MeshState
 {
   f3    N, T, B, Ng;
@@ -142,6 +153,8 @@
   f4    baseColorVertexMul;
   TexCtx tex;
   uint4 core0;
+  const PT_LDS_AS DevTexRef* refsLds    = nullptr;
+  uint32_t                   numRefsLds = 0;
 };
 PT_DEV bool isTexturePresent(uint16_t t) { return t > 0; }
 PT_DEV f4 fetchTexelRef(const TexCtx& tc, const DevTexRef& R, uint32_t levelOffset, int w, int x, int y)
@@ -286,12 +299,8 @@
   return R;
 #endif
 }
-__device__ __noinline__ f4 getTextureRef(TexCtx tc, uint32_t slot, f2 tc0, f2 tc1, float texGrad)
-{
-#ifdef MI_PT_DIAG_NO_TEX
-  return mk4(0.5f + 1e-3f * (tc0.x + tc1.y + texGrad + float(slot)));
-#endif
-  const DevTexRef R  = loadTexRef(tc.refs, slot);
+PT_DEV f4 textureOfRef(const TexCtx& tc, const DevTexRef& R, f2 tc0, f2 tc1, float texGrad)
+{
   f2              t  = R.texCoord == 0 ? tc0 : tc1;
   const float*    U  = R.uv;
   f2              uv = texUv(U, t);
@@ -322,6 +331,33 @@
   f4 b = sampleLevelRef(tc, R, uv, l1, R.minFilter);
   return levelBlend(a, b, f);
 }
+__device__ __noinline__ f4 getTextureRef(TexCtx tc, uint32_t slot, f2 tc0, f2 tc1, float texGrad)
+{
+#ifdef MI_PT_DIAG_NO_TEX
+  return mk4(0.5f + 1e-3f * (tc0.x + tc1.y + texGrad + float(slot)));
+#endif
+  const DevTexRef R = loadTexRef(tc.refs, slot);
+  return textureOfRef(tc, R, tc0, tc1, texGrad);
+}
+PT_DEV DevTexRef loadTexRefLds(const PT_LDS_AS DevTexRef* refs, uint32_t slot)
+{
+  typedef const PT_LDS_AS uint32_t* LdsWordPtr;
+  LdsWordPtr p = (LdsWordPtr)(refs + slot);
+  DevTexRef  R;
+  uint32_t*  W = reinterpret_cast<uint32_t*>(&R);
+#pragma unroll
+  for(int k = 0; k < int(sizeof(DevTexRef) / 4); ++k)
+    W[k] = p[k];
+  return R;
+}
+__device__ __noinline__ f4 getTextureRefLds(TexCtx tc, const PT_LDS_AS DevTexRef* refsLds, uint32_t numLds, uint32_t slot, f2 tc0, f2 tc1, float texGrad)
+{
+#ifdef MI_PT_DIAG_NO_TEX
+  return mk4(0.5f + 1e-3f * (tc0.x + tc1.y + texGrad + float(slot)));
+#endif
+  const DevTexRef R = slot < numLds ? loadTexRefLds(refsLds, slot) : loadTexRef(tc.refs, slot);
+  return textureOfRef(tc, R, tc0, tc1, texGrad);
+}
 #ifndef MI_PT_CORE_TEX_BATCH
 #define MI_PT_CORE_TEX_BATCH 1
 #endif
@@ -438,14 +474,15 @@
   roughness = mk2(r * r, r * r);
   return baseColor;
 }
-template <bool SIMPLE, bool CORE = false>
-PT_DEV PbrMaterial evaluateMaterial(const DevScene& sc, const MiGltfShadeMaterial& m, const MeshState& st, unsigned& taps)
-{
-#define TEX(slot) (++taps, getTextureRef(st.tex, slot, st.tc0, st.tc1, st.texGrad))
+template <bool SIMPLE, bool CORE = false, bool LDS = false, class Mat = MiGltfShadeMaterial>
+PT_DEV PbrMaterial evaluateMaterial(const DevScene& sc, const Mat& m, const MeshState& st, unsigned& taps)
+{
+#define TEX(slot) (++taps, LDS ? getTextureRefLds(st.tex, st.refsLds, st.numRefsLds, slot, st.tc0, st.tc1, st.texGrad) : getTextureRef(st.tex, slot, st.tc0, st.tc1, st.texGrad))
   PbrMaterial p = defaultPbrMaterial();
   static_assert(offsetof(MiGltfShadeMaterial, pbrBaseColorTexture) % 8 == 0 && offsetof(MiGltfShadeMaterial, occlusionTexture) == offsetof(MiGltfShadeMaterial, pbrBaseColorTexture) + 8,
                 "core texture slots: base colour, normal, metallic-roughness, emissive, occlusion");
-  const uint32_t* slotWords = reinterpret_cast<const uint32_t*>(&m.pbrBaseColorTexture);
+  typedef typename PtrLike<uint32_t, Mat>::type SlotWordPtr;
+  SlotWordPtr     slotWords = (SlotWordPtr)(&m.pbrBaseColorTexture);
   const uint32_t  sw0 = slotWords[0], sw1 = slotWords[1], sw2 = slotWords[2];
   const uint16_t  texBaseColor = uint16_t(sw0 & 0xffffu), texNormal = uint16_t(sw0 >> 16), texMetallicRoughness = uint16_t(sw1 & 0xffffu),
                  texEmissive = uint16_t(sw1 >> 16), texOcclusion = uint16_t(sw2 & 0xffffu);
@@ -462,7 +499,7 @@
   {
     f4    diffuse    = mk4(m.pbrDiffuseFactor[0], m.pbrDiffuseFactor[1], m.pbrDiffuseFactor[2], m.pbrDiffuseFactor[3]) * st.baseColorVertexMul;
     float glossiness = m.pbrGlossinessFactor;
-    f3    specular   = mk3(m.pbrSpecularFactor);
+    f3    specular   = mk3p(&m.pbrSpecularFactor[0]);
     if(isTexturePresent(m.pbrDiffuseTexture))
       diffuse *= TEX(m.pbrDiffuseTexture);
     if(isTexturePresent(m.pbrSpecularGlossinessTexture))
@@ -511,19 +548,19 @@
     p.N                = normalize(st.T * nv.x + st.B * nv.y + st.N * nv.z);
     needsTangentUpdate = true;
   }
-  p.emissive = mk3(m.emissiveFactor);
+  p.emissive = mk3p(&m.emissiveFactor[0]);
   if(isTexturePresent(texEmissive))
     p.emissive *= xyz(TEX(texEmissive));
   p.emissive            = max3(mk3(0.0f), p.emissive);
   if(!SIMPLE)
   {
-    p.attenuationColor    = mk3(m.attenuationColor);
+    p.attenuationColor    = mk3p(&m.attenuationColor[0]);
     p.attenuationDistance = m.attenuationDistance;
     p.thickness           = m.thicknessFactor;
     if(isTexturePresent(m.thicknessTexture))
       p.thickness *= TEX(m.thicknessTexture).y;
   }
-  p.specularColor = mk3(m.specularColorFactor);
+  p.specularColor = mk3p(&m.specularColorFactor[0]);
   if(isTexturePresent(m.specularColorTexture))
     p.specularColor *= xyz(TEX(m.specularColorTexture));
   p.specular = m.specularFactor;
@@ -543,7 +580,7 @@
   p.transmission = m.transmissionFactor;
   if(isTexturePresent(m.transmissionTexture))
     p.transmission *= TEX(m.transmissionTexture).x;
-  f3 ms = mk3(m.multiscatterColorFactor);
+  f3 ms = mk3p(&m.multiscatterColorFactor[0]);
   if(ms.x > 0.0f || ms.y > 0.0f || ms.z > 0.0f)
   {
     f3 ssa               = multiToSingleScatterAlbedo(ms);
@@ -603,7 +640,7 @@
   }
   if(!SIMPLE)
   {
-  p.sheenColor = mk3(m.sheenColorFactor);
+  p.sheenColor = mk3p(&m.sheenColorFactor[0]);
   if(isTexturePresent(m.sheenColorTexture))
     p.sheenColor *= xyz(TEX(m.sheenColorTexture));
   p.sheenRoughness = m.sheenRoughnessFactor;
@@ -614,7 +651,7 @@
   p.diffuseTransmissionFactor = m.diffuseTransmissionFactor;
   if(isTexturePresent(m.diffuseTransmissionTexture))
     p.diffuseTransmissionFactor *= TEX(m.diffuseTransmissionTexture).w;
-  p.diffuseTransmissionColor = mk3(m.diffuseTransmissionColor);
+  p.diffuseTransmissionColor = mk3p(&m.diffuseTransmissionColor[0]);
   if(isTexturePresent(m.diffuseTransmissionColorTexture))
     p.diffuseTransmissionColor *= xyz(TEX(m.diffuseTransmissionColorTexture));
   p.retroreflection = m.retroreflectionFactor;
diff --git a/vk_gltf_renderer_amd/pathtracer.py b/vk_gltf_renderer_amd/pathtracer.py
--- a/vk_gltf_renderer_amd/pathtracer.py
+++ b/vk_gltf_renderer_amd/pathtracer.py
@@ -294,6 +294,11 @@
         _check_pt(self._l.mi_pt_get_accel_resident_info(self._p, C.byref(a)))
         return {n: getattr(a, n) for n, _ in a._fields_}
 
+    def shade_lds_info(self):
+        a = capi.MiPtShadeLdsInfo()
+        _check_pt(self._l.mi_pt_get_shade_lds_info(self._p, C.byref(a)))
+        return {n: getattr(a, n) for n, _ in a._fields_ if n != "reserved"}
+
     def read_vertices(self, prim):
         p = self._scene.desc.contents.renderPrimitives[prim]
         n = int(p.vertexCount)
```

New measurement: 754.2. No clear change (-0.9%).
